# Strong-AI-Lab/ct-vae

Measured on AMD Instinct MI355X. Metric: images/sec/GPU fwd+bwd, 64×64×3 bs=64; recon+KL vs CPU ref, higher is better.
Workload: dtype f32; 1 GPU; VanillaVAE 64x64x3 train step fwd+loss+bwd+Adam (configs/vae.yaml shapes at the batch BASELINE.json's metric names, bs=64, on one MI355X; BASELINE.json configs[1..4] are the `configs` entries); per_gpu_batch=64, global_batch=64, latent_dim=128, parallelism=single, hipgraph=True, allreduce_overlap=False

## Files before the change

ct-vae_amd/csrc/api.hip:

```cpp
#include "../../include/ctvae_hip.h"

#include "common.hpp"
#include "gatlayer.hpp"
#include "glinear.hpp"
#include "pair.hpp"

namespace ctvae {
int launch_tapgemm(const ConvGeom& g, const float* G, const float* W, const float* bias, const float* add,
                   const float* mask, int mask_act, float* S, int act, float* bn_part, float* ws, size_t ws_floats,
                   hipStream_t st, const BnBwdFuse* bnb = nullptr, const InXform* xf = nullptr,
                   const WinoFilters* wf = nullptr, SplitKRaw* raw = nullptr, int out_pix = 0);
bool out_pix_supported(const ConvGeom& g, size_t ws_floats, int out_pix);
bool wino_supported(const ConvGeom& g, size_t ws_floats);
bool wino_enabled();
int wino_set_enabled(int on);
int launch_crop_resize_u8(const unsigned char* img, const long long* rows, float* out, int B, int N, int H, int W, int crop,
                          int S, hipStream_t st);
bool thin_forward_supported(const ConvGeom& g);
bool thin_wgrad_supported(const ConvGeom& g);
int tapgemm_bnb_rows(const ConvGeom& g, size_t ws_floats);
bool img_dgrad_supported(const ConvGeom& g);
void tapgemm_plan(const ConvGeom& g, size_t ws_floats, TapGemmPlan& p);
int launch_wgrad(const ConvGeom& g, const float* X, const float* dY, float* dW, float* dbias, float* ws, size_t ws_bytes,
                 int accumulate, hipStream_t st, const InXform* xf = nullptr, const DyXform* dyx = nullptr);
// ... 338 lines not shown
  const InXform xf{in_scale, in_shift, in_act};
  const InXform* xfp = in_scale != nullptr ? &xf : nullptr;
  if (!a_out && !scale_shift_out) return kErrBadArg;
  if (training && (!save_mean || !save_invstd)) return kErrBadArg;
  if (!training && (!running_mean || !running_var)) return kErrBadArg;
  if (Co % 4 != 0) return kErrBadArg;
  ConvGeom g;
  if (conv_geom(g, kind, 0, B, H, W, Ci, Co, k, stride, pad, out_pad)) return kErrBadArg;
  const size_t wsf = ws_bytes / sizeof(float);
  TapGemmPlan plan;
  tapgemm_plan(g, wsf, plan);
  const int R = g.B * g.sH * g.sW;
  if (plan.splitk > 1 || !training) {
    SplitKRaw raw{ws, 0};
    const bool fused = training && plan.splitk > 1 && bn_fused_ok(R, Co);
    int rc = launch_tapgemm(g, x, w, bias, nullptr, nullptr, 0, y, ACT_NONE, nullptr, ws, wsf, (hipStream_t)stream, nullptr, xfp,
                            nullptr, fused ? &raw : nullptr);
    if (rc) return rc;
    if (raw.splitk > 1) {
      const BnFusedFwd p{ws, row_map_of(g), raw.splitk, R, Co, bias, gamma, beta, running_mean, running_var, momentum, eps, save_mean, save_invstd,
                         scale_shift_out, nbt, y, a_out, act};
      return launch_bn_fused_forward(p, (hipStream_t)stream);
    }
    return launch_bn_forward(y, R, Co, gamma, beta, running_mean, running_var, momentum, eps, training, act, a_out, save_mean,
                             save_invstd, ws, ws_bytes, nbt, (hipStream_t)stream, scale_shift_out);
  }
  const int nparts = plan.bn_parts;
  if (wsf < bn_workspace_floats(Co, nparts)) return kErrWorkspace;
  int rc = launch_tapgemm(g, x, w, bias, nullptr, nullptr, 0, y, ACT_NONE, ws, nullptr, 0, (hipStream_t)stream, nullptr, xfp);
  if (rc) return rc;
  return launch_bn_finish_forward(y, R, Co, nparts, gamma, beta, running_mean, running_var, momentum, eps, training, act,
                                  a_out, save_mean, save_invstd, ws, nbt, (hipStream_t)stream, scale_shift_out);
}

int ctvae_conv_dgrad(int kind, const float* dy, const float* w, const float* add, const float* mask, int mask_act,
                     float* dx, int B, int H, int W, int Ci, int Co, int k, int stride, int pad, int out_pad,
                     const float* wino_filters, float* ws, size_t ws_bytes, void* stream) {
  if (!dy || !w || !dx || !conv_kind_ok(kind)) return kErrBadArg;
  ConvGeom g;
  if (conv_geom(g, kind, 2, B, H, W, Ci, Co, k, stride, pad, out_pad)) return kErrBadArg;
  if (wino_filters != nullptr && !ctvae_conv_wino_filter_floats(kind, B, H, W, Ci, Co, k, stride, pad, out_pad, ws_bytes))
    return kErrBadArg;
  const WinoFilters wf{wino_filters, nullptr};
  return launch_tapgemm(g, dy, w, nullptr, add, mask, mask_act, dx, ACT_NONE, nullptr, ws, ws_bytes / sizeof(float),
                        (hipStream_t)stream, nullptr, nullptr, &wf);
}

int ctvae_conv_wgrad(int kind, const float* x, const float* dy, float* dw, float* dbias, int B, int H, int W, int Ci,
                     int Co, int k, int stride, int pad, int out_pad, int accumulate, const float* in_scale,
                     const float* in_shift, int in_act, const float* dy_bn_y, const float* dy_bn_coef, int dy_bn_act,
                     float* gy_out, float* bn_dgamma, float* bn_dbeta, int bn_accumulate, float* ws, size_t ws_bytes,
                     void* stream) {
  if (!x || !dy || !dw || !ws || !conv_kind_ok(kind)) return kErrBadArg;
  if ((in_scale != nullptr) != (in_shift != nullptr)) return kErrBadArg;
  if ((dy_bn_y != nullptr) != (dy_bn_coef != nullptr) || (gy_out != nullptr && dy_bn_y == nullptr)) return kErrBadArg;
  if ((bn_dgamma != nullptr) != (bn_dbeta != nullptr) || (bn_dgamma != nullptr && (dy_bn_y == nullptr || gy_out != nullptr)))
    return kErrBadArg;
  ConvGeom g;
  if (conv_geom(g, kind, 0, B, H, W, Ci, Co, k, stride, pad, out_pad)) return kErrBadArg;
  const InXform xf{in_scale, in_shift, in_act};
  const DyXform dyx{dy_bn_y, dy_bn_coef, gy_out, dy_bn_act, bn_dgamma, bn_dbeta, bn_accumulate};
  float* wws = defer_wgrad_ws(ws, ws_bytes / sizeof(float));
  const int rc = launch_wgrad(g, x, dy, dw, dbias, wws, ws_bytes, accumulate, (hipStream_t)stream, &xf, &dyx);
  defer_wgrad_done();
  return rc;
}

int ctvae_defer_begin(float* arena, size_t arena_bytes) { return defer_begin(arena, arena_bytes / sizeof(float)); }
int ctvae_defer_flush(void* stream) { return defer_flush((hipStream_t)stream); }

int ctvae_conv_backward_bn_rows(int kind, int B, int H, int W, int Ci, int Co, int k, int stride, int pad, int out_pad,
                                size_t ws_bytes) {
  if (!conv_kind_ok(kind)) return 0;
  ConvGeom g;
  if (conv_geom(g, kind, 2, B, H, W, Ci, Co, k, stride, pad, out_pad)) return 0;
  PairCtx ctx;
  pair_ctx() = &ctx;
  const int rows = tapgemm_bnb_rows(g, ((ws_bytes / 2) & ~(size_t)255) / sizeof(float));
  pair_ctx() = nullptr;
  return rows;
}

static thread_local int g_lazy_pixel_major = 0;

static int conv_backward_impl(int kind, const float* x, const float* dy, const float* w, float* dw, float* dbias, float* dx, int B,
                        int H, int W, int Ci, int Co, int k, int stride, int pad, int out_pad, int accumulate, const float* mask,
                        int mask_act, const float* wino_filters, const float* bn_y, const float* bn_mean,
                        const float* bn_invstd, const float* bn_gamma, const float* bn_beta, int bn_act, float* bn_part,
                        int bn_part_rows, float* bn_coef_out, float* bn_dgamma, float* bn_dbeta, int bn_accumulate,
                        const float* in_scale, const float* in_shift, int in_act,
                        const float* dy_bn_y, const float* dy_bn_coef, int dy_bn_act, float* gy_out, float* ws, size_t ws_bytes,
                        void* stream, float* dx_slices) {
  if (!x || !dy || !w || !dw || (!dx && !dx_slices) || !ws || !conv_kind_ok(kind)) return kErrBadArg;
  const bool bn = bn_part != nullptr;
  if (bn_coef_out != nullptr && !bn) return kErrBadArg;
  if ((bn_dgamma != nullptr) != (bn_dbeta != nullptr) || (bn_dgamma != nullptr && bn_coef_out == nullptr)) return kErrBadArg;
  if ((in_scale != nullptr) != (in_shift != nullptr)) return kErrBadArg;
  if ((dy_bn_y != nullptr) != (dy_bn_coef != nullptr) || (dy_bn_y != nullptr) != (gy_out != nullptr)) return kErrBadArg;
  if (bn && (!bn_y || !bn_mean || !bn_invstd || !bn_gamma || !bn_beta)) return kErrBadArg;
  ConvGeom gw, gd;
  if (conv_geom(gw, kind, 0, B, H, W, Ci, Co, k, stride, pad, out_pad)) return kErrBadArg;
  if (conv_geom(gd, kind, 2, B, H, W, Ci, Co, k, stride, pad, out_pad)) return kErrBadArg;
  const size_t half_bytes = (ws_bytes / 2) & ~(size_t)255, half_floats = half_bytes / sizeof(float);
  float* ws_d = ws + half_floats;
  if (wino_filters != nullptr && !ctvae_conv_wino_filter_floats(kind, B, H, W, Ci, Co, k, stride, pad, out_pad, half_bytes))
    return kErrBadArg;
  const hipStream_t st = (hipStream_t)stream;
  PairCtx ctx;
  pair_ctx() = &ctx;
  if (bn) {
    const int rows = tapgemm_bnb_rows(gd, half_floats);
    if (rows <= 0 || rows != bn_part_rows || (img_dgrad_supported(gd) && mask != nullptr)) {
      pair_ctx() = nullptr;
      return kErrBadArg;
    }
  }
  {
    TapGemmPlan pl;
    tapgemm_plan(gd, half_floats, pl);
    ctx.dgrad_wgs = (long)pl.mtiles * pl.ntiles * gd.ncls * (pl.splitk > 1 ? pl.splitk : 1);
    int kmax = 0;
    for (int c = 0; c < gd.ncls; ++c) kmax = gd.ntaps[c] * gd.gC / KC > kmax ? gd.ntaps[c] * gd.gC / KC : kmax;
    ctx.dgrad_chunks = pl.splitk > 1 ? (kmax + pl.splitk - 1) / pl.splitk : kmax;
  }
  const InXform xf{in_scale, in_shift, in_act};
  const DyXform dyx{dy_bn_y, dy_bn_coef, gy_out, dy_bn_act};
  int rc;
  if (bn && bn_act != ACT_TANH && x == bn_y && in_scale != nullptr && in_act == bn_act && mask == nullptr && dy_bn_y == nullptr &&
      img_conv_supported(gw) && img_dgrad_supported(gd) && img_backward_fused_ws_floats(gd) <= half_floats) {
    float *part = nullptr, *pb = nullptr;
    int np = 0;
    const BnBwdFuse f{bn_y, bn_mean, bn_invstd, bn_gamma, bn_beta, bn_act, bn_part};
    rc = launch_img_backward_fused(gd, dy, w, dx, &f, ws, &part, &pb, &np, dbias != nullptr, st);
    if (!rc) rc = wgrad_finish_slabs(part, dw, 9L * 32 * 3, np, pb, dbias, 3L, accumulate, st);
  } else {
    float* wws = bn_coef_out == nullptr ? defer_wgrad_ws(ws, half_floats) : ws;
    rc = launch_wgrad(gw, x, dy, dw, dbias, wws, half_bytes, accumulate, st, &xf, &dyx);
    defer_wgrad_done();
    if (!rc) {
    const WinoFilters wf{wino_filters, nullptr};
    const BnBwdFuse f{bn_y, bn_mean, bn_invstd, bn_gamma, bn_beta, bn_act, bn_part};
      SplitKRaw raw{dx_slices, 0, g_lazy_pixel_major};
      g_lazy_pixel_major = 0;
      rc = launch_tapgemm(gd, gy_out != nullptr ? gy_out : dy, w, nullptr, nullptr, mask, mask_act, dx, ACT_NONE, nullptr, ws_d,
                          half_floats, st, bn ? &f : nullptr, nullptr, &wf, dx_slices != nullptr ? &raw : nullptr);
      if (!rc && dx_slices != nullptr && raw.splitk <= 1) rc = kErrBadArg;
    }
  }
  pair_ctx() = nullptr;
  if (rc) return rc;
  if (bn_coef_out != nullptr) {
    ctx.haveBF = true;
    ctx.bf = BnFinJob{bn_part, bn_part_rows, Ci, (float)((long)B * H * W), bn_gamma, bn_mean, bn_invstd, bn_beta, bn_coef_out,
                      bn_dgamma, bn_dbeta, bn_accumulate};
  }
  return pair_flush(ctx, st);
}

int ctvae_conv_backward(int kind, const float* x, const float* dy, const float* w, float* dw, float* dbias, float* dx, int B,
                        int H, int W, int Ci, int Co, int k, int stride, int pad, int out_pad, int accumulate, const float* mask,
                        int mask_act, const float* wino_filters, const float* bn_y, const float* bn_mean,
                        const float* bn_invstd, const float* bn_gamma, const float* bn_beta, int bn_act, float* bn_part,
                        int bn_part_rows, float* bn_coef_out, float* bn_dgamma, float* bn_dbeta, int bn_accumulate,
                        const float* in_scale, const float* in_shift, int in_act,
                        const float* dy_bn_y, const float* dy_bn_coef, int dy_bn_act, float* gy_out, float* ws, size_t ws_bytes,
                        void* stream) {
  return conv_backward_impl(kind, x, dy, w, dw, dbias, dx, B, H, W, Ci, Co, k, stride, pad, out_pad, accumulate, mask, mask_act,
                            wino_filters, bn_y, bn_mean, bn_invstd, bn_gamma, bn_beta, bn_act, bn_part, bn_part_rows, bn_coef_out,
                            bn_dgamma, bn_dbeta, bn_accumulate, in_scale, in_shift, in_act, dy_bn_y, dy_bn_coef, dy_bn_act, gy_out, ws,
                            ws_bytes, stream, nullptr);
}

int ctvae_conv_backward_lazy_slices(int kind, int B, int H, int W, int Ci, int Co, int k, int stride, int pad, int out_pad,
                                    int for_bn, size_t ws_bytes) {
  if (!conv_kind_ok(kind)) return 0;
  ConvGeom g;
  if (conv_geom(g, kind, 2, B, H, W, Ci, Co, k, stride, pad, out_pad)) return 0;
  const size_t half_floats = ((ws_bytes / 2) & ~(size_t)255) / sizeof(float);
  if (img_dgrad_supported(g) || (wino_enabled() && wino_supported(g, half_floats))) return 0;
  PairCtx ctx;
  pair_ctx() = &ctx;
  TapGemmPlan pl;
  tapgemm_plan(g, half_floats, pl);
  pair_ctx() = nullptr;
  const long Mc = (long)g.B * g.Qh * g.Qw;
  if (pl.thin || pl.splitk <= 1) return 0;
  if (for_bn && (Mc % 4 != 0 || !bn_fused_ok(B * H * W, Ci))) return 0;
  return pl.splitk;
}

int ctvae_conv_backward_lazy(int kind, const float* x, const float* dy, const float* w, float* dw, float* dbias, float* dx_slices,
                             int B, int H, int W, int Ci, int Co, int k, int stride, int pad, int out_pad, int accumulate,
                             const float* in_scale, const float* in_shift, int in_act, int pixel_major, float* ws, size_t ws_bytes,
                             void* stream) {
  if (!dx_slices) return kErrBadArg;
  g_lazy_pixel_major = pixel_major;
  return conv_backward_impl(kind, x, dy, w, dw, dbias, nullptr, B, H, W, Ci, Co, k, stride, pad, out_pad, accumulate, nullptr, 0,
                            nullptr, nullptr, nullptr, nullptr, nullptr, nullptr, 0, nullptr, 0, nullptr, nullptr, nullptr, 0, in_scale,
                            in_shift, in_act, nullptr, nullptr, 0, nullptr, ws, ws_bytes, stream, dx_slices);
}

int ctvae_bn_backward_fused(const float* g_a_slices, int slices, int kind, int B, int H, int W, int Ci, int Co, int k, int stride,
                            int pad, int out_pad, const float* y, const float* gamma, const float* beta, const float* save_mean,
                            const float* save_invstd, int act, float* g_y, float* dgamma, float* dbeta, int accumulate, void* stream) {
  if (!g_a_slices || slices < 1 || !y || !gamma || !beta || !save_mean || !save_invstd || !g_y || !dgamma || !dbeta) return kErrBadArg;
  if (!conv_kind_ok(kind)) return kErrBadArg;
  ConvGeom g;
  if (conv_geom(g, kind, 2, B, H, W, Ci, Co, k, stride, pad, out_pad)) return kErrBadArg;
  const BnFusedBwd p{g_a_slices, row_map_of(g), slices, B * H * W, Ci, y, gamma, beta, save_mean, save_invstd, act, g_y, dgamma,
                     dbeta, accumulate};
  return launch_bn_fused_backward(p, (hipStream_t)stream);
}

int ctvae_conv_wgrad_bn_apply_supported(int kind, int B, int H, int W, int Ci, int Co, int k, int stride, int pad, int out_pad) {
  if (!conv_kind_ok(kind)) return 0;
  ConvGeom g;
  if (conv_geom(g, kind, 0, B, H, W, Ci, Co, k, stride, pad, out_pad)) return 0;
  if (upconv_wgrad_supported(g)) return 1;
  return img_enc_supported(g) ? 2 : 0;
}

int ctvae_bn_forward(const float* y, int R, int C, const float* gamma, const float* beta, float* running_mean,
                     float* running_var, float momentum, float eps, int training, int act, float* out,
                     float* save_mean, float* save_invstd, int64_t* num_batches_tracked, float* ws, size_t ws_bytes,
                     void* stream) {
  if (!y || !gamma || !beta || !out || !ws) return kErrBadArg;
  if (training && (!save_mean || !save_invstd)) return kErrBadArg;
  if (!training && (!running_mean || !running_var)) return kErrBadArg;
  return launch_bn_forward(y, R, C, gamma, beta, running_mean, running_var, momentum, eps, training, act, out, save_mean,
                           save_invstd, ws, ws_bytes, (long long*)num_batches_tracked, (hipStream_t)stream);
}

int ctvae_bn_backward(const float* g_a, const float* beta, const float* y, int R, int C, const float* gamma,
                      const float* save_mean, const float* save_invstd, int act, float* g_y, float* dgamma,
                      float* dbeta, int accumulate, const float* part_in, int part_rows, float* coef_out,
                      const float* coef_in, float* ws, size_t ws_bytes, void* stream) {
  if (!g_a || !beta || !y || !gamma || !save_mean || !save_invstd || !dgamma || !dbeta || !ws) return kErrBadArg;
  if (!g_y && !coef_out) return kErrBadArg;
  if ((part_in != nullptr) != (part_rows > 0)) return kErrBadArg;
  if (coef_in != nullptr && (!g_y || part_in != nullptr || coef_out != nullptr)) return kErrBadArg;
  return launch_bn_backward(g_a, beta, y, R, C, gamma, save_mean, save_invstd, act, g_y, dgamma, dbeta, accumulate, ws,
                            ws_bytes, part_in, part_rows, (hipStream_t)stream, coef_out, coef_in);
}

int ctvae_gat_score(int mode, const float* xl, const float* xr, const float* attr, const float* we, const float* att, float* out,
                    int B, int N, int H, int C, float slope, void* stream) {
  if (!xl || !xr || !attr || !we || !att || !out || (mode != 0 && mode != 1)) return kErrBadArg;
  return launch_gat_score(mode, xl, xr, attr, we, att, out, B, N, H, C, slope, (hipStream_t)stream);
}

int ctvae_gat_score_backward(const float* xl, const float* xr, const float* attr, const float* we, const float* att,
                             const float* g, float* d_xl, float* d_xr, float* d_att_part, float* d_we_part, int B, int N, int H,
                             int C, float slope, void* stream) {
  if (!xl || !xr || !attr || !we || !att || !g || !d_xl || !d_xr || !d_att_part || !d_we_part) return kErrBadArg;
  return launch_gat_score_backward(xl, xr, attr, we, att, g, d_xl, d_xr, d_att_part, d_we_part, B, N, H, C, slope,
// ... 678 lines not shown
```

ct-vae_amd/csrc/common.hpp:

```cpp
#pragma once
#include <hip/hip_runtime.h>
#include <stdint.h>
#include <stdio.h>
#include <string.h>

#include "geom.hpp"

namespace ctvae {

typedef float f32x2 __attribute__((ext_vector_type(2)));
typedef float f32x4 __attribute__((ext_vector_type(4)));
typedef float f32x16 __attribute__((ext_vector_type(16)));

constexpr float kLeaky = 0.01f;

enum Act : int { ACT_NONE = 0, ACT_LRELU = 1, ACT_RELU = 2, ACT_TANH = 3 };

__device__ __forceinline__ float act_fwd(float v, int act) {
  switch (act) {
    case ACT_LRELU: return v > 0.f ? v : v * kLeaky;
    case ACT_RELU: return v > 0.f ? v : 0.f;
    case ACT_TANH: return 1.f - 2.f * __frcp_rn(__expf(2.f * v) + 1.f);
    default: return v;
  }
// ... 31 lines not shown
}

__device__ __forceinline__ double wave_sum_d_full(double v) {
#define CTVAE_DPP_D(CTRL, RM, BC)                                                                          \
  {                                                                                                        \
    const long long b = __builtin_bit_cast(long long, v);                                                  \
    const int lo = __builtin_amdgcn_update_dpp(0, (int)b, CTRL, RM, 0xF, BC);                               \
    const int hi = __builtin_amdgcn_update_dpp(0, (int)(b >> 32), CTRL, RM, 0xF, BC);                       \
    v += __builtin_bit_cast(double, ((long long)hi << 32) | (unsigned)lo);                                 \
  }
  CTVAE_DPP_D(0xB1, 0xF, true)
  CTVAE_DPP_D(0x4E, 0xF, true)
  CTVAE_DPP_D(0x141, 0xF, true)
  CTVAE_DPP_D(0x140, 0xF, true)
  CTVAE_DPP_D(0x142, 0xA, false)
  CTVAE_DPP_D(0x143, 0xC, false)
#undef CTVAE_DPP_D
  const long long b = __builtin_bit_cast(long long, v);
  const int lo = __builtin_amdgcn_readlane((int)b, 63), hi = __builtin_amdgcn_readlane((int)(b >> 32), 63);
  return __builtin_bit_cast(double, ((long long)hi << 32) | (unsigned)lo);
}

__device__ __forceinline__ double wave_sum_d(double v) {
#pragma unroll
  for (int o = 32; o > 0; o >>= 1) v += __shfl_xor(v, o, 64);
  return v;
}

__device__ __forceinline__ float block_sum_256(float v, float* sm ) {
  v = wave_sum_full(v);
  const int w = threadIdx.x >> 6;
  __syncthreads();
  if ((threadIdx.x & 63) == 0) sm[w] = v;
  __syncthreads();
  return sm[0] + sm[1] + sm[2] + sm[3];
}

inline int ceil_div(int a, int b) { return (a + b - 1) / b; }

template <int BYTES>
__device__ __forceinline__ void kernarg_warm() {
#if defined(__HIP_DEVICE_COMPILE__)
  const void* ka = __builtin_amdgcn_kernarg_segment_ptr();
  unsigned junk;
  asm volatile(
      ".set .Lkw_off, 0\n"
      ".rept %2\n"
      "s_load_dword %0, %1, .Lkw_off\n"
      ".set .Lkw_off, .Lkw_off + 64\n"
      ".endr\n"
      "s_waitcnt lgkmcnt(0)"
      : "=&s"(junk)
      : "s"(ka), "n"((BYTES + 63) / 64)
      : "memory");
#endif
}
template <int BYTES, int O0, int O1, int O2>
__device__ __forceinline__ void kernarg_warm_get(int& v0, int& v1, int& v2) {
#if defined(__HIP_DEVICE_COMPILE__)
  const void* ka = __builtin_amdgcn_kernarg_segment_ptr();
  unsigned junk;
  asm volatile(
      "s_load_dword %1, %4, %6\n"
      "s_load_dword %2, %4, %7\n"
      "s_load_dword %3, %4, %8\n"
      ".set .Lkw_off, 0\n"
      ".rept %5\n"
      "s_load_dword %0, %4, .Lkw_off\n"
      ".set .Lkw_off, .Lkw_off + 64\n"
      ".endr\n"
      "s_waitcnt lgkmcnt(0)"
      : "=&s"(junk), "=&s"(v0), "=&s"(v1), "=&s"(v2)
      : "s"(ka), "n"((BYTES + 63) / 64), "n"(O0), "n"(O1), "n"(O2)
      : "memory");
#endif
}

struct InXform {
  const float* scale;
  const float* shift;
  int act;
};

struct DyXform {
  const float* y;
  const float* coef;
  float* gy_out;
  int act;
  float* dgamma = nullptr;
  float* dbeta = nullptr;
  int bn_accumulate = 0;
};

struct WinoFilters {
  const float* ready;
  float* bwd_out;
};

struct BnBwdFuse {
  const float* y;
  const float* mean;
  const float* invstd;
  const float* gamma;
  const float* beta;
  int act;
  float* part;
};

struct SplitKRaw {
  float* part;
  int splitk;
  int pixel_major = 0;
};

struct RowMap {
  int ncls, Mc, Qh, Qw, sH, sW, os;
  unsigned pyp, pxp;
  int lgMc, lgQhw, lgQw;
};

inline RowMap row_map_of(const ConvGeom& g) {
  RowMap m{};
  m.ncls = g.ncls; m.Mc = g.B * g.Qh * g.Qw; m.Qh = g.Qh; m.Qw = g.Qw; m.sH = g.sH; m.sW = g.sW; m.os = g.os;
  static_assert(kMaxCls <= 4, "RowMap packs four classes");
  for (int c = 0; c < kMaxCls; ++c) { m.pyp |= (unsigned)(g.py[c] & 0xff) << (8 * c); m.pxp |= (unsigned)(g.px[c] & 0xff) << (8 * c); }
  auto lg2 = [](int v) { int l = 0; while ((1 << l) < v) ++l; return (v > 0 && (1 << l) == v) ? l : -1; };
  m.lgMc = lg2(m.Mc); m.lgQhw = lg2(g.Qh * g.Qw); m.lgQw = lg2(g.Qw);
  if (m.lgMc < 0 || m.lgQhw < 0 || m.lgQw < 0) m.lgMc = m.lgQhw = m.lgQw = -1;
  return m;
}

__device__ __forceinline__ int row_map_pixel(const RowMap& m, int r) {
  if (m.ncls == 1) return r;
  int cls, b, qy, qx;
  if (m.lgMc >= 0) {
    cls = r >> m.lgMc;
    const int mm = r & (m.Mc - 1);
    b = mm >> m.lgQhw;
    const int rr = mm & ((1 << m.lgQhw) - 1);
    qy = rr >> m.lgQw;
    qx = rr & (m.Qw - 1);
  } else {
    cls = r / m.Mc;
    const int mm = r - cls * m.Mc;
    const int qhw = m.Qh * m.Qw;
    b = mm / qhw;
    const int rr = mm - b * qhw;
    qy = rr / m.Qw;
    qx = rr - qy * m.Qw;
  }
  const int py = (int)((m.pyp >> (8 * cls)) & 0xffu), px = (int)((m.pxp >> (8 * cls)) & 0xffu);
  return (b * m.sH + qy * m.os + py) * m.sW + qx * m.os + px;
}

struct TapGemmPlan {
  int BM, BN, mtiles, ntiles, splitk;
  int thin;
  int bn_parts;
};

#define CTVAE_LAUNCH_CHECK()                   \
  do {                                         \
    hipError_t e__ = hipGetLastError();        \
    if (e__ != hipSuccess) return (int)e__;    \
  } while (0)

constexpr int kErrBadArg = -22;
constexpr int kErrWorkspace = -12;

}
```

ct-vae_amd/csrc/image.hip:

```cpp
#include <type_traits>

#include "common.hpp"
#include "prof.hpp"

namespace ctvae {

#ifdef CTVAE_PHASE_TIMING
__device__ unsigned long long g_img_phase[1024 * 32];
#define IPHASE(i) do { if (threadIdx.x == 0 && blockIdx.x < 1024 && (i) < 32) g_img_phase[blockIdx.x * 32 + (i)] = wall_clock64(); } while (0)
extern "C" int ctvae_debug_img_phase_read(unsigned long long* out, int n) {
  return (int)hipMemcpyFromSymbol(out, HIP_SYMBOL(g_img_phase), (size_t)n * 8);
}
#else
#define IPHASE(i) do {} while (0)
#endif

namespace {

constexpr int TH = 8, TW = 32, PH = 10, PW = 34, NP = PH * PW , NPP = 352 ;
constexpr int LDA = 36;
constexpr int GH = 12, GW = 36;
constexpr int C = 32, NO = 3, NT = 9, NJ = 27;
constexpr unsigned kOOBi = 0x80000000u;

// ... 397 lines not shown
  auto g_load = [&](const TileXY& t) {
#pragma unroll
    for (int j = 0; j < 2; ++j) {
      const int pp = tid + 256 * j;
      const int py = (pp * 241) >> 13, px = pp - py * PW;
      const int iy = t.y0 - 1 + py, ix = t.x0 - 1 + px;
      const bool ok = pp < NP && (unsigned)iy < (unsigned)a.H && (unsigned)ix < (unsigned)a.W;
      const unsigned off = ok ? (unsigned)(((t.b * a.H + iy) * a.W + ix) * NO) * 4u : kOOBi;
#pragma unroll
      for (int n = 0; n < NO; ++n) gq[j][n] = ld1(rG, ok ? off + 4u * n : kOOBi);
    }
  };
  int tile = blockIdx.x;
  TileXY cur = tile_xy(a, tile < a.ntiles ? tile : 0);
  if (tile < a.ntiles) g_load(cur);
  for (; tile < a.ntiles; tile += gridDim.x) {
#pragma unroll
    for (int j = 0; j < 2; ++j) {
      const int pp = tid + 256 * j;
      if (pp < NP)
#pragma unroll
        for (int n = 0; n < NO; ++n) sG[pp * 4 + n] = gq[j][n];
    }
    __syncthreads();
    const int next = tile + gridDim.x;
    const TileXY nxt = tile_xy(a, next < a.ntiles ? next : 0);
    if (next < a.ntiles) g_load(nxt);
#pragma unroll
    for (int i = 0; i < 2; ++i) {
      const int ly = wave + 4 * i;
      const unsigned rowoff = (unsigned)(((cur.b * a.H + cur.y0 + ly) * a.W + cur.x0) * C + li) * 4u;
      float yv[16];
      if (bn) {
#pragma unroll
        for (int r = 0; r < 16; ++r) yv[r] = ld1(rY, rowoff + (unsigned)((8 * (r >> 2) + 4 * lh + (r & 3)) * C) * 4u);
      }
      f32x16 acc;
#pragma unroll
      for (int r = 0; r < 16; ++r) acc[r] = 0.f;
      const float* gp = &sG[((ly + 1) * PW + li + 1) * 4];
#pragma unroll
      for (int s = 0; s < 14; ++s) acc = __builtin_amdgcn_mfma_f32_32x32x2f32(gp[koff[s]], bw[s], acc, 0, 0, 0);
#pragma unroll
      for (int r = 0; r < 16; ++r) st1(rO, rowoff + (unsigned)((8 * (r >> 2) + 4 * lh + (r & 3)) * C) * 4u, acc[r]);
      if (bn) {
        if (a.bn_act == ACT_TANH) {
#pragma unroll
          for (int r = 0; r < 16; ++r) {
            const float xh = (yv[r] - bmean) * binv;
            const float g1 = acc[r] * act_bwd_from_out(act_fwd(bgm * xh + bbt, ACT_TANH), ACT_TANH);
            s1 += g1;
            s2 += g1 * xh;
          }
        } else {
          const float bsl = act_slope(a.bn_act);
#pragma unroll
          for (int r = 0; r < 16; ++r) {
            const float xh = (yv[r] - bmean) * binv;
            const float g1 = acc[r] * act_slope_bwd(bgm * xh + bbt, bsl);
            s1 += g1;
            s2 += g1 * xh;
          }
        }
      }
    }
    __syncthreads();
    cur = nxt;
  }
  if (bn) {
    s1 += __shfl_xor(s1, 32, 64);
    s2 += __shfl_xor(s2, 32, 64);
    if (lh == 0) {
      sS[(wave * C + li) * 2] = s1;
      sS[(wave * C + li) * 2 + 1] = s2;
    }
    __syncthreads();
    if (tid < C * 2) {
      const float v = ((sS[tid] + sS[C * 2 + tid]) + sS[2 * C * 2 + tid]) + sS[3 * C * 2 + tid];
      a.bn_part[(long)blockIdx.x * C * 2 + tid] = v;
    }
  }
}

__global__ __launch_bounds__(256, 4) void img_bwd_fused_kernel(const ImgArgs a, float* __restrict__ wpart, float* __restrict__ wpbias) {
  kernarg_warm<sizeof(ImgArgs) + 16>();
  const float bn_slope = act_slope(a.bn_act);
  __shared__ __attribute__((aligned(16))) float sG[NP * 4];
  __shared__ __attribute__((aligned(16))) float sR[4 * 32 * 32];
  __shared__ float sS[4 * C * 2];
  __shared__ float sB[4 * NO];
  const int tid = threadIdx.x, lane = tid & 63, wave = tid >> 6, li = lane & 31, lh = lane >> 5;
  const __amdgpu_buffer_rsrc_t rG = rsrc(a.dY, (long)a.B * a.H * a.W * NO * 4);
  const long obytes = (long)a.B * a.H * a.W * C * 4;
  const __amdgpu_buffer_rsrc_t rO = rsrc(a.out, obytes);
  const __amdgpu_buffer_rsrc_t rY = rsrc(a.bn_y, obytes);

  int koff[14];
  float bw[14];
#pragma unroll
  for (int s = 0; s < 14; ++s) {
    const int k0 = 2 * s, k1 = 2 * s + 1;
    const int t0 = k0 / 3, c0 = k0 % 3, t1 = (k1 < NJ ? k1 : 0) / 3, c1 = (k1 < NJ ? k1 : 0) % 3;
    const int o0 = (a.tdy[t0] * PW + a.tdx[t0]) * 4 + c0, o1 = (a.tdy[t1] * PW + a.tdx[t1]) * 4 + c1;
    const float w0 = a.Wt[(a.twt[t0] * C + li) * NO + c0];
    const float w1 = k1 < NJ ? a.Wt[(a.twt[t1] * C + li) * NO + c1] : 0.f;
    koff[s] = lh ? (k1 < NJ ? o1 : 0) : o0;
    bw[s] = lh ? w1 : w0;
  }
  const int jj = li < NJ ? li : NJ - 1;
  const int t_l = jj / 3, co_l = jj - 3 * t_l;
  const int wlane = ((1 + tap_dy(a, t_l)) * PW + (1 + tap_dx(a, t_l)) + 4 * lh) * 4 + co_l;
  const float bmean = a.bn_mean[li], binv = a.bn_invstd[li], bgm = a.bn_gamma[li], bbt = a.bn_beta[li];
  float s1 = 0.f, s2 = 0.f;
  float bs[NO] = {0.f, 0.f, 0.f};
  f32x16 wacc;
#pragma unroll
  for (int r = 0; r < 16; ++r) wacc[r] = 0.f;

  float gq[2][NO];
  auto g_load = [&](const TileXY& t) {
#pragma unroll
    for (int j = 0; j < 2; ++j) {
      const int pp = tid + 256 * j;
      const int py = (pp * 241) >> 13, px = pp - py * PW;
      const int iy = t.y0 - 1 + py, ix = t.x0 - 1 + px;
      const bool ok = pp < NP && (unsigned)iy < (unsigned)a.H && (unsigned)ix < (unsigned)a.W;
      const unsigned off = ok ? (unsigned)(((t.b * a.H + iy) * a.W + ix) * NO) * 4u : kOOBi;
#pragma unroll
      for (int n = 0; n < NO; ++n) gq[j][n] = ld1(rG, ok ? off + 4u * n : kOOBi);
    }
  };
  int tile = blockIdx.x;
  TileXY cur = tile_xy(a, tile < a.ntiles ? tile : 0);
  if (tile < a.ntiles) g_load(cur);
  for (; tile < a.ntiles; tile += gridDim.x) {
#pragma unroll
    for (int j = 0; j < 2; ++j) {
      const int pp = tid + 256 * j;
      if (pp < NP) {
        const int py = (pp * 241) >> 13, px = pp - py * PW;
        const bool inner = py >= 1 && py <= TH && px >= 1 && px <= TW;
#pragma unroll
        for (int n = 0; n < NO; ++n) {
          sG[pp * 4 + n] = gq[j][n];
          bs[n] += inner ? gq[j][n] : 0.f;
        }
      }
    }
    __syncthreads();
    const int next = tile + gridDim.x;
    const TileXY nxt = tile_xy(a, next < a.ntiles ? next : 0);
    if (next < a.ntiles) g_load(nxt);
#pragma unroll 1
    for (int i = 0; i < 2; ++i) {
      const int ly = wave + 4 * i;
      const unsigned rowoff = (unsigned)(((cur.b * a.H + cur.y0 + ly) * a.W + cur.x0) * C + li) * 4u;
      float yv[16];
#pragma unroll
      for (int r = 0; r < 16; ++r) yv[r] = ld1(rY, rowoff + (unsigned)((8 * (r >> 2) + 4 * lh + (r & 3)) * C) * 4u);
      f32x16 acc;
#pragma unroll
      for (int r = 0; r < 16; ++r) acc[r] = 0.f;
      const float* gp = &sG[((ly + 1) * PW + li + 1) * 4];
#pragma unroll
      for (int s = 0; s < 14; ++s) acc = __builtin_amdgcn_mfma_f32_32x32x2f32(gp[koff[s]], bw[s], acc, 0, 0, 0);
#pragma unroll
      for (int r = 0; r < 16; ++r) st1(rO, rowoff + (unsigned)((8 * (r >> 2) + 4 * lh + (r & 3)) * C) * 4u, acc[r]);
      const float* gw = &sG[ly * PW * 4 + wlane];
#pragma unroll
      for (int r = 0; r < 16; ++r) {
        const float xh = (yv[r] - bmean) * binv;
        const float t = bgm * xh + bbt;
        const float av = act_slope_fwd(t, bn_slope);
        const float g1 = acc[r] * act_slope_bwd(t, bn_slope);
        s1 += g1;
        s2 += g1 * xh;
        wacc = __builtin_amdgcn_mfma_f32_32x32x2f32(av, gw[(8 * (r >> 2) + (r & 3)) * 4], wacc, 0, 0, 0);
      }
    }
    __syncthreads();
    cur = nxt;
  }
  s1 += __shfl_xor(s1, 32, 64);
  s2 += __shfl_xor(s2, 32, 64);
  if (lh == 0) {
    sS[(wave * C + li) * 2] = s1;
    sS[(wave * C + li) * 2 + 1] = s2;
  }
#pragma unroll
  for (int r = 0; r < 16; ++r) sR[(wave * 32 + 8 * (r >> 2) + 4 * lh + (r & 3)) * 32 + li] = wacc[r];
  float bwv[NO];
#pragma unroll
  for (int n = 0; n < NO; ++n) bwv[n] = wave_sum(bs[n]);
  if (lane == 0)
#pragma unroll
    for (int n = 0; n < NO; ++n) sB[wave * NO + n] = bwv[n];
  __syncthreads();
  if (tid < C * 2) {
    const float v = ((sS[tid] + sS[C * 2 + tid]) + sS[2 * C * 2 + tid]) + sS[3 * C * 2 + tid];
    a.bn_part[(long)blockIdx.x * C * 2 + tid] = v;
  }
  for (int e = tid; e < C * NJ; e += 256) {
    const int ci = e / NJ, j = e - ci * NJ;
    const float v = ((sR[(0 * 32 + ci) * 32 + j] + sR[(1 * 32 + ci) * 32 + j]) + sR[(2 * 32 + ci) * 32 + j]) + sR[(3 * 32 + ci) * 32 + j];
    const int t = j / 3, co = j - 3 * t;
    wpart[((long)blockIdx.x * (NT * C) + tap_wt(a, t) * C + ci) * NO + co] = v;
  }
  if (wpbias != nullptr && tid < NO) wpbias[(long)blockIdx.x * NO + tid] = ((sB[tid] + sB[NO + tid]) + sB[2 * NO + tid]) + sB[3 * NO + tid];
}

constexpr int EPH = 2 * TH + 1, EPW = 2 * TW + 1, ENP = EPH * EPW;
constexpr int ENLD = (ENP + 255) / 256;

struct EncArgs {
  const float* X;
  const float* Wt;
  const float* bias;
  const float* dY;
  float* out;
  float* pbias;
  float* bn_part;
  const float* dy_y;
  const float* dy_coef;
  float* dgamma;
  float* dbeta;
  int dy_act, bn_accumulate;
  int act;
  int B, H, W, tiles_y, tiles_x, ntiles;
  int tdy[NT], tdx[NT], twt[NT];
};

struct EncPatch {
  float v[ENLD][NO];
};

__device__ __forceinline__ void enc_patch_load(const EncArgs& a, __amdgpu_buffer_rsrc_t rX, const TileXY& t, EncPatch& p) {
  const int IH = 2 * a.H, IW = 2 * a.W;
#pragma unroll
  for (int j = 0; j < ENLD; ++j) {
    const int pp = threadIdx.x + 256 * j;
    const int py = (pp * 1009) >> 16, px = pp - py * EPW;
    const int iy = 2 * t.y0 - 1 + py, ix = 2 * t.x0 - 1 + px;
    const bool ok = pp < ENP && (unsigned)iy < (unsigned)IH && (unsigned)ix < (unsigned)IW;
    const unsigned off = (unsigned)(((t.b * IH + iy) * IW + ix) * NO) * 4u;
#pragma unroll
    for (int n = 0; n < NO; ++n) p.v[j][n] = ld1(rX, ok ? off + 4u * n : kOOBi);
  }
}
__device__ __forceinline__ void enc_patch_store(const EncPatch& p, float* sX) {
#pragma unroll
// ... 246 lines not shown
  ProfScope ps("img_enc_fwd_kernel", st, 2.0 * a.ntiles * TH * TW * NT * C * NO, 4.0 * a.ntiles * TH * TW * (C + 4 * NO));
  hipLaunchKernelGGL(img_enc_fwd_kernel, dim3(img_enc_rows(g)), dim3(256), 0, st, a);
  CTVAE_LAUNCH_CHECK();
  return 0;
}

int launch_img_enc_wgrad(const ConvGeom& g, const float* X, const float* dY, float* ws, float** part_out, float** pbias_out,
                         int* nparts, bool want_bias, hipStream_t st, const DyXform* dyx) {
  EncArgs a{};
  fill_enc(a, g);
  a.X = X; a.dY = dY;
  if (dyx != nullptr && dyx->y != nullptr) {
    if (dyx->gy_out != nullptr || (dyx->act != ACT_NONE && dyx->act != ACT_RELU && dyx->act != ACT_LRELU)) return kErrBadArg;
    if ((dyx->dgamma != nullptr) != (dyx->dbeta != nullptr)) return kErrBadArg;
    a.dy_y = dyx->y; a.dy_coef = dyx->coef; a.dy_act = dyx->act;
    a.dgamma = dyx->dgamma; a.dbeta = dyx->dbeta; a.bn_accumulate = dyx->bn_accumulate;
  }
  const int nwg = a.ntiles < 512 ? a.ntiles : 512;
  a.out = ws;
  a.pbias = want_bias ? ws + (size_t)nwg * NJ * C : nullptr;
  ProfScope ps("img_enc_wgrad_kernel", st, 2.0 * a.ntiles * TH * TW * NT * C * NO, 4.0 * a.ntiles * TH * TW * (C + 4 * NO));
  if (a.dy_y != nullptr) hipLaunchKernelGGL(img_enc_wgrad_kernel<true>, dim3(nwg), dim3(256), 0, st, a);
  else hipLaunchKernelGGL(img_enc_wgrad_kernel<false>, dim3(nwg), dim3(256), 0, st, a);
  CTVAE_LAUNCH_CHECK();
  *part_out = a.out;
  *pbias_out = a.pbias;
  *nparts = nwg;
  return 0;
}

constexpr int kImgFwd2Wgs = 1024, kImgWgradWgs = 512, kImgDgradWgs = 1024;

int img_wgrad_parts(const ConvGeom& g) {
  const int nt = g.B * (g.sH / TH) * (g.sW / TW);
  return nt < kImgWgradWgs ? nt : kImgWgradWgs;
}
int img_dgrad_rows(const ConvGeom& g) {
  const int nt = g.B * (g.sH / TH) * (g.sW / TW);
  return nt < kImgDgradWgs ? nt : kImgDgradWgs;
}

int launch_img_forward(const ConvGeom& g, const float* X, const float* W, const float* bias, float* S, int act,
                       const InXform* xf, hipStream_t st) {
  ImgArgs a{};
  fill(a, g);
  a.X = X; a.Wt = W; a.bias = bias; a.out = S; a.act = act;
  if (xf != nullptr && xf->scale != nullptr) { a.scale = xf->scale; a.shift = xf->shift; a.in_act = xf->act; }
  ProfScope ps("img_fwd_kernel", st, 2.0 * a.ntiles * TH * TW * NT * C * NO, 4.0 * a.ntiles * TH * TW * (C + NO));
  const int nwg = a.ntiles < kImgFwd2Wgs ? a.ntiles : kImgFwd2Wgs;
  hipLaunchKernelGGL(img_fwd2_kernel, dim3(nwg), dim3(256), 0, st, a);
  CTVAE_LAUNCH_CHECK();
  return 0;
}

int launch_img_wgrad(const ConvGeom& g, const float* X, const float* dY, float* ws, float** part_out, float** pbias_out,
                     int* nparts, bool want_bias, const InXform* xf, hipStream_t st) {
  ImgArgs a{};
  fill(a, g);
  a.X = X; a.dY = dY;
  if (xf != nullptr && xf->scale != nullptr) { a.scale = xf->scale; a.shift = xf->shift; a.in_act = xf->act; }
  const int nwg = img_wgrad_parts(g);
  a.out = ws;
  a.pbias = want_bias ? ws + (size_t)nwg * NT * C * NO : nullptr;
  ProfScope ps("img_wgrad_kernel", st, 2.0 * a.ntiles * TH * TW * NT * C * NO, 4.0 * a.ntiles * TH * TW * (C + NO));
  hipLaunchKernelGGL(img_wgrad_kernel, dim3(nwg), dim3(256), 0, st, a);
  CTVAE_LAUNCH_CHECK();
  *part_out = a.out;
  *pbias_out = a.pbias;
  *nparts = nwg;
  return 0;
}

int launch_img_backward_fused(const ConvGeom& g, const float* dY, const float* W, float* dX, const BnBwdFuse* bnb, float* ws,
                              float** part_out, float** pbias_out, int* nparts, bool want_bias, hipStream_t st) {
  if (bnb->act == ACT_TANH) return kErrBadArg;
  ImgArgs a{};
  fill(a, g);
  a.dY = dY; a.Wt = W; a.out = dX;
  a.bn_y = bnb->y; a.bn_mean = bnb->mean; a.bn_invstd = bnb->invstd; a.bn_gamma = bnb->gamma; a.bn_beta = bnb->beta;
  a.bn_act = bnb->act; a.bn_part = bnb->part;
  const int nwg = img_dgrad_rows(g);
  float* part = ws;
  float* pb = want_bias ? ws + (size_t)nwg * NT * C * NO : nullptr;
  ProfScope ps("img_bwd_fused_kernel", st, 4.0 * a.ntiles * TH * TW * NT * C * NO, 4.0 * a.ntiles * TH * TW * (C * 2 + NO));
  hipLaunchKernelGGL(img_bwd_fused_kernel, dim3(nwg), dim3(256), 0, st, a, part, pb);
  CTVAE_LAUNCH_CHECK();
  *part_out = part;
  *pbias_out = pb;
  *nparts = nwg;
  return 0;
}
size_t img_backward_fused_ws_floats(const ConvGeom& g) { return (size_t)img_dgrad_rows(g) * (NT * C * NO + NO); }

int launch_img_dgrad(const ConvGeom& g, const float* dY, const float* W, float* dX, const BnBwdFuse* bnb, hipStream_t st) {
  ImgArgs a{};
  fill(a, g);
  a.dY = dY; a.Wt = W; a.out = dX;
  if (bnb != nullptr && bnb->part != nullptr) {
    a.bn_y = bnb->y; a.bn_mean = bnb->mean; a.bn_invstd = bnb->invstd; a.bn_gamma = bnb->gamma; a.bn_beta = bnb->beta;
    a.bn_act = bnb->act; a.bn_part = bnb->part;
  }
  const int nwg = img_dgrad_rows(g);
  ProfScope ps("img_dgrad_kernel", st, 2.0 * a.ntiles * TH * TW * NT * C * NO,
               4.0 * a.ntiles * TH * TW * (C * (a.bn_part != nullptr ? 2 : 1) + NO));
  hipLaunchKernelGGL(img_dgrad_kernel, dim3(nwg), dim3(256), 0, st, a);
  CTVAE_LAUNCH_CHECK();
  return 0;
}

}
```

ct-vae_amd/csrc/upconv.hip:

```cpp
#include "common.hpp"
#include "phase.hpp"
#include <type_traits>

#include "prof.hpp"

namespace ctvae {

namespace {

constexpr int TH = 8, TW = 32, PH = 9, PW = 33, NP = PH * PW ;
constexpr int LDA = 36, C = 32, NT = 9, NCLS = 4, MAXT = 4;
constexpr int NLD = (NP * 8 + 255) / 256;
constexpr unsigned kOOBu = 0x80000000u;

struct UpArgs {
  const float* X;
  const float* Wt;
  const float* bias;
  const float* dY;
  float* out;
  float* pbias;
  float* bn_part;
  const float* dy_y;
  const float* dy_coef;
  float* gy_out;
  int dy_act;
  const float* xf_scale;
  const float* xf_shift;
  int xf_act;
  int act;
  int B, H, W, tiles_y, tiles_x, ntiles;
  int ntaps[NCLS], cpy[NCLS], cpx[NCLS];
  int tdy[NCLS][MAXT], tdx[NCLS][MAXT], twt[NCLS][MAXT];
};

__device__ __forceinline__ f32x4 ld4(__amdgpu_buffer_rsrc_t r, unsigned off) {
  return __builtin_bit_cast(f32x4, __builtin_amdgcn_raw_buffer_load_b128(r, (int)off, 0, 0));
}
__device__ __forceinline__ float ld1(__amdgpu_buffer_rsrc_t r, unsigned off) {
  return __builtin_bit_cast(float, __builtin_amdgcn_raw_buffer_load_b32(r, (int)off, 0, 0));
}
__device__ __forceinline__ void st1(__amdgpu_buffer_rsrc_t r, unsigned off, float v) {
  __builtin_amdgcn_raw_buffer_store_b32(__builtin_bit_cast(unsigned, v), r, (int)off, 0, 0);
}
__device__ __forceinline__ __amdgpu_buffer_rsrc_t rsrc(const void* p, long bytes) {
  return __builtin_amdgcn_make_buffer_rsrc(const_cast<void*>(p), 0, (int)bytes, 0x00020000);
}

struct TileXY {
  int b, y0, x0;
};
__device__ __forceinline__ TileXY tile_xy(const UpArgs& a, int tile) {
  const int per = a.tiles_y * a.tiles_x;
  const int b = tile / per, r = tile - b * per;
  const int ty = r / a.tiles_x;
  return TileXY{b, ty * TH, (r - ty * a.tiles_x) * TW};
}

struct Patch {
  f32x4 v[NLD];
};
__device__ __forceinline__ void patch_load(const UpArgs& a, __amdgpu_buffer_rsrc_t rX, const TileXY& t, Patch& p) {
#pragma unroll
  for (int j = 0; j < NLD; ++j) {
    const int e = threadIdx.x + 256 * j;
    const int pp = e >> 3, c4 = e & 7;
    const int py = (pp * 1986) >> 16, px = pp - py * PW;
    const int iy = t.y0 + py, ix = t.x0 + px;
    const bool ok = e < NP * 8 && iy < a.H && ix < a.W;
    p.v[j] = ld4(rX, ok ? (unsigned)(((t.b * a.H + iy) * a.W + ix) * C + 4 * c4) * 4u : kOOBu);
  }
}
__device__ __forceinline__ void patch_store(const Patch& p, float* sA) {
#pragma unroll
  for (int j = 0; j < NLD; ++j) {
    const int e = threadIdx.x + 256 * j;
    if (e < NP * 8) *reinterpret_cast<f32x4*>(&sA[(e >> 3) * LDA + 4 * (e & 7)]) = p.v[j];
  }
}
__device__ __forceinline__ void patch_store_xf(const UpArgs& a, const TileXY& t, const Patch& p, float* sA, f32x4 sc, f32x4 sh,
                                               float nslope) {
#pragma unroll
  for (int j = 0; j < NLD; ++j) {
    const int e = threadIdx.x + 256 * j;
    const int pp = e >> 3;
    const int py = (pp * 1986) >> 16, px = pp - py * PW;
    const float inside = (t.y0 + py < a.H && t.x0 + px < a.W) ? 1.f : 0.f;
    f32x4 v = p.v[j];
#pragma unroll
    for (int q = 0; q < 4; ++q) {
      const float u = v[q] * sc[q] + sh[q] * inside;
      v[q] = fmaxf(u, u * nslope);
    }
    if (e < NP * 8) *reinterpret_cast<f32x4*>(&sA[pp * LDA + 4 * (e & 7)]) = v;
  }
}

CTVAE_PHASE_DECL(up)
__global__ __launch_bounds__(256, 2) void up_fwd_kernel(const UpArgs a) {
  CTVAE_PH(up, 0, 0);
  kernarg_warm<sizeof(UpArgs)>();
  extern __shared__ __attribute__((aligned(16))) float smem[];
  float* sA = smem;
  float* sW = smem + NP * LDA;
  __shared__ float sS[4 * C * 3];
  const int tid = threadIdx.x, lane = tid & 63, wave = tid >> 6, li = lane & 31, lh = lane >> 5;
  const __amdgpu_buffer_rsrc_t rX = rsrc(a.X, (long)a.B * a.H * a.W * C * 4);
  const int OH = 2 * a.H, OW = 2 * a.W;
  const __amdgpu_buffer_rsrc_t rO = rsrc(a.out, (long)a.B * OH * OW * C * 4);
// ... 78 lines not shown
    auto zero = [](f32x16& acc) {
#pragma unroll
      for (int r = 0; r < 16; ++r) acc[r] = 0.f;
    };
#define UP_STEP(LY, C_, T_, CUR, NXT, NLY, NC, NT_, HAS_NEXT)          \
    if (HAS_NEXT) read_tap(NLY, NC, NT_, NXT);                          \
    mfma_tap(CUR, acc);                                                 \
    _Pragma("unroll") for (int g_ = 0; g_ < 16; ++g_) {                 \
      __builtin_amdgcn_sched_group_barrier(0x008, 1, 0);                \
      __builtin_amdgcn_sched_group_barrier(0x100, 2, 0);                \
    }                                                                   \
    __builtin_amdgcn_sched_barrier(0);
    Frag fa, fb;
#pragma unroll 1
    for (int i = 0; i < 2; ++i) {
      const int ly = wave + 4 * i;
      f32x16 acc;
      read_tap(ly, 0, 0, fa);
      zero(acc);
      UP_STEP(ly, 0, 0, fa, fb, ly, 1, 0, true)
      epilogue(ly, 0, acc);
      zero(acc);
      UP_STEP(ly, 1, 0, fb, fa, ly, 1, 1, true)
      UP_STEP(ly, 1, 1, fa, fb, ly, 2, 0, true)
      epilogue(ly, 1, acc);
      zero(acc);
      UP_STEP(ly, 2, 0, fb, fa, ly, 2, 1, true)
      UP_STEP(ly, 2, 1, fa, fb, ly, 3, 0, true)
      epilogue(ly, 2, acc);
      zero(acc);
      UP_STEP(ly, 3, 0, fb, fa, ly, 3, 1, true)
      UP_STEP(ly, 3, 1, fa, fb, ly, 3, 2, true)
      UP_STEP(ly, 3, 2, fb, fa, ly, 3, 3, true)
      UP_STEP(ly, 3, 3, fa, fb, ly, 0, 0, false)
      epilogue(ly, 3, acc);
    }
#undef UP_STEP
    CTVAE_PH(up, 0, 3);
    __syncthreads();
    CTVAE_PH(up, 0, 4);
    cur = nxt;
  }
  if (a.bn_part != nullptr) {
    {
      const float on = __shfl_xor(sn, 32, 64), om = __shfl_xor(smean, 32, 64), oq = __shfl_xor(sm2, 32, 64);
      const float ntot = sn + on;
      if (ntot > 0.f) {
        const float d = om - smean;
        sm2 = sm2 + oq + d * d * (sn * on / ntot);
        smean = smean + d * (on / ntot);
      }
      sn = ntot;
    }
    if (lh == 0) {
      float* st = &sS[(wave * C + li) * 3];
      st[0] = sn; st[1] = smean; st[2] = sm2;
    }
    __syncthreads();
    if (tid < C) {
      float n = 0.f, mean = 0.f, m2 = 0.f;
#pragma unroll
      for (int w = 0; w < 4; ++w) {
        const float nb = sS[(w * C + tid) * 3], mb = sS[(w * C + tid) * 3 + 1], qb = sS[(w * C + tid) * 3 + 2];
        if (nb > 0.f) {
          const float ntot = n + nb, d = mb - mean;
          mean += d * (nb / ntot);
          m2 += qb + d * d * (n * nb / ntot);
          n = ntot;
        }
      }
      float* p = a.bn_part + ((long)blockIdx.x * C + tid) * 3;
      p[0] = n; p[1] = mean; p[2] = m2;
    }
  }
}


template <int CLS>
struct ClsInfo {
  static constexpr int ntaps = CLS == 0 ? 1 : (CLS == 3 ? 4 : 2);
  static constexpr int first = CLS == 0 ? 0 : (CLS == 1 ? 1 : (CLS == 2 ? 3 : 5));
};

template <bool FUSED>
__global__ __launch_bounds__(256, 1) void up_wgrad_kernel(const UpArgs a) {
  kernarg_warm<sizeof(UpArgs)>();
  __shared__ __attribute__((aligned(16))) float sA[NP * LDA];
  __shared__ __attribute__((aligned(16))) float sR[4 * C * C];
  __shared__ float sB[4 * C];
  const int tid = threadIdx.x, lane = tid & 63, wave = tid >> 6, li = lane & 31, lh = lane >> 5;
  const __amdgpu_buffer_rsrc_t rX = rsrc(a.X, (long)a.B * a.H * a.W * C * 4);
  const int OH = 2 * a.H, OW = 2 * a.W;
  const long obytes = (long)a.B * OH * OW * C * 4;
  const __amdgpu_buffer_rsrc_t rG = rsrc(a.dY, obytes);
  const __amdgpu_buffer_rsrc_t rYb = rsrc(a.dy_y, FUSED ? obytes : 0);
  const __amdgpu_buffer_rsrc_t rGY = rsrc(a.gy_out, FUSED ? obytes : 0);
  const float k1 = FUSED ? a.dy_coef[li] : 0.f, k2 = FUSED ? a.dy_coef[C + li] : 0.f, k3 = FUSED ? a.dy_coef[2 * C + li] : 0.f;
  const float ksc = FUSED ? a.dy_coef[3 * C + li] : 0.f, ksh = FUSED ? a.dy_coef[4 * C + li] : 0.f;
  const float nslope = a.dy_act == ACT_LRELU ? kLeaky : (a.dy_act == ACT_RELU ? 0.f : 1.f);
  const bool xf = a.xf_scale != nullptr;
  const f32x4 xsc = xf ? *reinterpret_cast<const f32x4*>(a.xf_scale + 4 * (tid & 7)) : f32x4{0.f, 0.f, 0.f, 0.f};
  const f32x4 xsh = xf ? *reinterpret_cast<const f32x4*>(a.xf_shift + 4 * (tid & 7)) : f32x4{0.f, 0.f, 0.f, 0.f};
  const float xns = a.xf_act == ACT_LRELU ? kLeaky : (a.xf_act == ACT_RELU ? 0.f : 1.f);

  f32x16 acc[NT];
#pragma unroll
  for (int t = 0; t < NT; ++t)
#pragma unroll
    for (int r = 0; r < 16; ++r) acc[t][r] = 0.f;
  float bsum = 0.f;

  CTVAE_PH(up, 1, 0);
  for (int tile = blockIdx.x; tile < a.ntiles; tile += gridDim.x) {
    const TileXY cur = tile_xy(a, tile);
    CTVAE_PH(up, 1, 1);
#pragma unroll
    for (int h = 0; h < 2; ++h) {
      f32x4 v[NLD / 2];
#pragma unroll
      for (int j = 0; j < NLD / 2; ++j) {
        const int e = tid + 256 * (j + h * (NLD / 2));
        const int pp = e >> 3, c4 = e & 7;
        const int py = (pp * 1986) >> 16, px = pp - py * PW;
        const int iy = cur.y0 + py, ix = cur.x0 + px;
        const bool ok = e < NP * 8 && iy < a.H && ix < a.W;
        v[j] = ld4(rX, ok ? (unsigned)(((cur.b * a.H + iy) * a.W + ix) * C + 4 * c4) * 4u : kOOBu);
      }
      if (xf) {
#pragma unroll
        for (int j = 0; j < NLD / 2; ++j) {
          const int e = tid + 256 * (j + h * (NLD / 2));
          const int pp = e >> 3;
          const int py = (pp * 1986) >> 16, px = pp - py * PW;
          const float inside = (cur.y0 + py < a.H && cur.x0 + px < a.W) ? 1.f : 0.f;
#pragma unroll
          for (int q = 0; q < 4; ++q) {
            const float u = v[j][q] * xsc[q] + xsh[q] * inside;
            v[j][q] = fmaxf(u, u * xns);
          }
        }
      }
#pragma unroll
      for (int j = 0; j < NLD / 2; ++j) {
        const int e = tid + 256 * (j + h * (NLD / 2));
        if (e < NP * 8) *reinterpret_cast<f32x4*>(&sA[(e >> 3) * LDA + 4 * (e & 7)]) = v[j];
      }
    }
    __syncthreads();

    CTVAE_PH(up, 1, 2);
    float dv[3][8], yv[FUSED ? 3 : 1][FUSED ? 8 : 1];
    auto step_off = [&](int ly, int c, int h) {
      return (unsigned)((((cur.b * OH + 2 * (cur.y0 + ly) + a.cpy[c]) * OW + 2 * cur.x0 + a.cpx[c] + 2 * (16 * h + lh)) * C + li)) * 4u;
    };
    auto dy_load = [&](unsigned off, auto slot_c) {
      constexpr int slot = decltype(slot_c)::value;
#pragma unroll
      for (int j = 0; j < 8; ++j) dv[slot][j] = ld1(rG, off + (unsigned)(4 * j * C) * 4u);
      if constexpr (FUSED) {
#pragma unroll
        for (int j = 0; j < 8; ++j) yv[slot][j] = ld1(rYb, off + (unsigned)(4 * j * C) * 4u);
      }
    };
    auto run_step = [&](int ly, auto cls_c, int h, unsigned off, auto slot_c) {
      constexpr int CLS = decltype(cls_c)::value;
      constexpr int slot = decltype(slot_c)::value;
      using CI = ClsInfo<CLS>;
      int xo[CI::ntaps];
#pragma unroll
      for (int t = 0; t < CI::ntaps; ++t) xo[t] = ((ly + a.tdy[CLS][t]) * PW + 16 * h + lh + a.tdx[CLS][t]) * LDA + li;
      float xa[CI::ntaps], xb[CI::ntaps];
#pragma unroll
      for (int t = 0; t < CI::ntaps; ++t) xa[t] = sA[xo[t]];
#pragma unroll
      for (int j = 0; j < 8; ++j) {
        if (j + 1 < 8) {
#pragma unroll
          for (int t = 0; t < CI::ntaps; ++t) xb[t] = sA[xo[t] + 2 * (j + 1) * LDA];
        }
        float d = dv[slot][j];
        if constexpr (FUSED) {
          const float yy = yv[slot][j];
          const float g1 = (yy * ksc + ksh) > 0.f ? d : d * nslope;
          d = k1 * g1 + k2 * yy + k3;
          st1(rGY, off + (unsigned)(4 * j * C) * 4u, d);
        }
        bsum += d;
#pragma unroll
        for (int t = 0; t < CI::ntaps; ++t)
          acc[CI::first + t] = __builtin_amdgcn_mfma_f32_32x32x2f32(xa[t], d, acc[CI::first + t], 0, 0, 0);
#pragma unroll
        for (int t = 0; t < CI::ntaps; ++t) xa[t] = xb[t];
        __builtin_amdgcn_sched_barrier(0);
      }
    };
    unsigned soff[3];
    auto issue = [&](auto s_c) {
      constexpr int S = decltype(s_c)::value;
      soff[S % 3] = step_off(wave + 4 * (S / 8), (S % 8) / 2, S & 1);
      dy_load(soff[S % 3], std::integral_constant<int, S % 3>{});
    };
    auto do_step = [&](auto s_c) {
      constexpr int S = decltype(s_c)::value;
      if constexpr (S + 2 < 16) issue(std::integral_constant<int, S + 2>{});
      run_step(wave + 4 * (S / 8), std::integral_constant<int, (S % 8) / 2>{}, S & 1, soff[S % 3], std::integral_constant<int, S % 3>{});
    };
    issue(std::integral_constant<int, 0>{});
    issue(std::integral_constant<int, 1>{});
#define UPW_STEP(S_) do_step(std::integral_constant<int, S_>{});
    UPW_STEP(0) UPW_STEP(1) UPW_STEP(2) UPW_STEP(3) UPW_STEP(4) UPW_STEP(5) UPW_STEP(6) UPW_STEP(7)
    CTVAE_PH(up, 1, 3);
    UPW_STEP(8) UPW_STEP(9) UPW_STEP(10) UPW_STEP(11) UPW_STEP(12) UPW_STEP(13) UPW_STEP(14) UPW_STEP(15)
#undef UPW_STEP
    CTVAE_PH(up, 1, 4);
    __syncthreads();
  }
  bsum += __shfl_xor(bsum, 32, 64);
  if (lh == 0) sB[wave * C + li] = bsum;
  auto merge_tap = [&](int wtap, const f32x16& v) {
    __syncthreads();
#pragma unroll
    for (int r = 0; r < 16; ++r) sR[(wave * C + 8 * (r >> 2) + 4 * lh + (r & 3)) * C + li] = v[r];
    __syncthreads();
    for (int e = tid; e < C * C; e += 256) {
      const float s4 = ((sR[e] + sR[C * C + e]) + sR[2 * C * C + e]) + sR[3 * C * C + e];
      a.out[((long)blockIdx.x * NT + wtap) * C * C + e] = s4;
    }
  };
  merge_tap(a.twt[0][0], acc[0]);
  merge_tap(a.twt[1][0], acc[1]);
  merge_tap(a.twt[1][1], acc[2]);
  merge_tap(a.twt[2][0], acc[3]);
  merge_tap(a.twt[2][1], acc[4]);
  merge_tap(a.twt[3][0], acc[5]);
  merge_tap(a.twt[3][1], acc[6]);
  merge_tap(a.twt[3][2], acc[7]);
  merge_tap(a.twt[3][3], acc[8]);
  if (a.pbias != nullptr && tid < C) a.pbias[(long)blockIdx.x * C + tid] = ((sB[tid] + sB[C + tid]) + sB[2 * C + tid]) + sB[3 * C + tid];
  CTVAE_PH(up, 1, 5);
}

void fill(UpArgs& a, const ConvGeom& g) {
  a.B = g.B; a.H = g.gH; a.W = g.gW;
  a.tiles_y = g.gH / TH; a.tiles_x = g.gW / TW;
  a.ntiles = g.B * a.tiles_y * a.tiles_x;
  for (int c = 0; c < NCLS; ++c) {
    a.ntaps[c] = g.ntaps[c]; a.cpy[c] = g.py[c]; a.cpx[c] = g.px[c];
    for (int t = 0; t < MAXT; ++t) {
      const bool ok = t < g.ntaps[c];
      a.tdy[c][t] = ok ? g.taps[c][t].dy : 0;
      a.tdx[c][t] = ok ? g.taps[c][t].dx : 0;
      a.twt[c][t] = ok ? g.taps[c][t].wtap : 0;
    }
  }
}

constexpr size_t kUpFwdSmem = (size_t)(NP * LDA + NT * C * C) * 4;

}

bool upconv_supported(const ConvGeom& g) {
  if (!packed_weights(g) || g.wT != 0 || g.gC != C || g.sC != C || g.wCi != C || g.wCo != C) return false;
  if (g.is != 1 || g.os != 2 || g.ncls != NCLS) return false;
  if (g.sH != 2 * g.gH || g.sW != 2 * g.gW || g.gH % TH != 0 || g.gW % TW != 0) return false;
  int total = 0;
  for (int c = 0; c < NCLS; ++c) {
    if (g.ntaps[c] < 1 || g.ntaps[c] > MAXT) return false;
    total += g.ntaps[c];
    for (int t = 0; t < g.ntaps[c]; ++t) {
      const Tap& tp = g.taps[c][t];
      if (tp.dy < 0 || tp.dy > 1 || tp.dx < 0 || tp.dx > 1 || tp.wtap < 0 || tp.wtap >= NT) return false;
    }
  }
  if (g.ntaps[0] != 1 || g.ntaps[1] != 2 || g.ntaps[2] != 2 || g.ntaps[3] != 4) return false;
  return total == NT && (long)g.B * g.sH * g.sW * C < (1L << 29);
}
bool upconv_wgrad_supported(const ConvGeom& g) { return upconv_supported(g); }

constexpr int kUpWgs = 512;
int upconv_rows(const ConvGeom& g) {
  const int nt = g.B * (g.gH / TH) * (g.gW / TW);
  return nt < kUpWgs ? nt : kUpWgs;
}

int launch_upconv_forward(const ConvGeom& g, const float* X, const float* W, const float* bias, float* S, int act,
                          float* bn_part, hipStream_t st, const InXform* xf) {
  UpArgs a{};
  fill(a, g);
  a.X = X; a.Wt = W; a.bias = bias; a.out = S; a.act = act; a.bn_part = bn_part;
  if (xf != nullptr && xf->scale != nullptr) {
    if (xf->act != ACT_NONE && xf->act != ACT_RELU && xf->act != ACT_LRELU) return kErrBadArg;
    a.xf_scale = xf->scale; a.xf_shift = xf->shift; a.xf_act = xf->act;
  }
  static bool attr_set = false;
  if (!attr_set) {
    (void)hipFuncSetAttribute(reinterpret_cast<const void*>(up_fwd_kernel), hipFuncAttributeMaxDynamicSharedMemorySize, (int)kUpFwdSmem);
    attr_set = true;
  }
  ProfScope ps("up_fwd_kernel", st, 2.0 * a.ntiles * TH * TW * NT * C * C, 4.0 * a.ntiles * TH * TW * C * 5.0);
  hipLaunchKernelGGL(up_fwd_kernel, dim3(upconv_rows(g)), dim3(256), kUpFwdSmem, st, a);
  CTVAE_LAUNCH_CHECK();
  return 0;
}

int launch_upconv_wgrad(const ConvGeom& g, const float* X, const float* dY, float* ws, float** part_out, float** pbias_out,
                        int* nparts, bool want_bias, hipStream_t st, const DyXform* dyx, const InXform* xf) {
  UpArgs a{};
  fill(a, g);
  a.X = X; a.dY = dY;
  if (xf != nullptr && xf->scale != nullptr) {
    if (xf->act != ACT_NONE && xf->act != ACT_RELU && xf->act != ACT_LRELU) return kErrBadArg;
    a.xf_scale = xf->scale; a.xf_shift = xf->shift; a.xf_act = xf->act;
  }
  if (dyx != nullptr && dyx->y != nullptr && dyx->act != ACT_NONE && dyx->act != ACT_RELU && dyx->act != ACT_LRELU) return kErrBadArg;
  if (dyx != nullptr && dyx->y != nullptr) { a.dy_y = dyx->y; a.dy_coef = dyx->coef; a.gy_out = dyx->gy_out; a.dy_act = dyx->act; }
  const int nwg = upconv_rows(g);
  a.out = ws;
  a.pbias = want_bias ? ws + (size_t)nwg * NT * C * C : nullptr;
  ProfScope ps("up_wgrad_kernel", st, 2.0 * a.ntiles * TH * TW * NT * C * C, 4.0 * a.ntiles * TH * TW * C * 5.0);
  if (a.dy_y != nullptr) hipLaunchKernelGGL(up_wgrad_kernel<true>, dim3(nwg), dim3(256), 0, st, a);
  else hipLaunchKernelGGL(up_wgrad_kernel<false>, dim3(nwg), dim3(256), 0, st, a);
  CTVAE_LAUNCH_CHECK();
  *part_out = a.out;
  *pbias_out = a.pbias;
  *nparts = nwg;
  return 0;
}

}
```

ct-vae_amd/csrc/wgrad.hip:

```cpp
#include "common.hpp"
#include "prof.hpp"
#include "finish.hpp"
#include "pair.hpp"
#include "wgrad_fast.hpp"

namespace ctvae {


template <int WK, int WN, bool XVEC, bool DVEC>
__global__ __launch_bounds__(256) void wgrad_kernel(const WgradArgs a) {
  kernarg_warm<sizeof(WgradArgs)>();
  __shared__ __attribute__((aligned(16))) float sXbuf[MC * WK * 32];
  __shared__ __attribute__((aligned(16))) float sDbuf[MC * WN * 32];
  __shared__ int sRowPix[2][MC];
  __shared__ int sRowYX[2][MC];
  __shared__ int sRowOut[2][MC];
  wgrad_plain_body<WK, WN, XVEC, DVEC>(a, sXbuf, sDbuf, sRowPix, sRowYX, sRowOut, blockIdx.x, blockIdx.y, gridDim.x, gridDim.y);
}

template <int WK, int WN, int TK, int TN, bool XF = false>
__global__ __launch_bounds__(256) void wgrad_fast_kernel(const WgradArgs a, int lgQw, int lgQhw, int lgC) {
  kernarg_warm<sizeof(WgradArgs) + 12>();
  constexpr int KT = WK * TK * 32, NT = WN * TN * 32;
  __shared__ __attribute__((aligned(16))) float sX[MC * KT];
// ... 243 lines not shown

static int finish_reduce(const float* p1, float* d1, long n1, int S1, long st1, const float* p2, float* d2, long n2, int S2, long st2,
                         int accumulate, hipStream_t st) {
  if (defer_record(p1, d1, n1, S1, st1, p2, d2, n2, S2, st2, accumulate, st)) return 0;
  if (PairCtx* pc = pair_ctx(); pc != nullptr && !pc->haveRed) {
    pc->j1 = ReduceJob{p1, d1, n1, S1, st1, 0, 0};
    pc->j2 = (p2 != nullptr && d2 != nullptr) ? ReduceJob{p2, d2, n2, S2, st2, 0, 0} : ReduceJob{nullptr, nullptr, 0, 0, 0, 0, 0};
    pc->nb1 = reduce_job_blocks(pc->j1);
    pc->nb2 = reduce_job_blocks(pc->j2);
    pc->accumulate = accumulate;
    pc->bytesRed = 4.0 * (double)(S1 + 1) * n1;
    pc->haveRed = pc->nb1 + pc->nb2 > 0;
    return 0;
  }
  ProfScope ps("reduce_partials_kernel", st, 0.0, 4.0 * (double)(S1 + 1) * n1);
  if (p2 != nullptr && d2 != nullptr) launch_reduce2(p1, d1, n1, S1, st1, p2, d2, n2, S2, st2, accumulate, st);
  else launch_reduce(p1, d1, n1, S1, st1, accumulate, st);
  CTVAE_LAUNCH_CHECK();
  return 0;
}

int wgrad_finish_slabs(const float* part, float* dW, long n, int nparts, const float* pbias, float* dbias, long nb, int accumulate,
                       hipStream_t st) {
  return finish_reduce(part, dW, n, nparts, n, pbias, dbias, nb, nparts, nb, accumulate, st);
}

size_t wgrad_workspace_floats(const ConvGeom& g, int S) {
  int taps_total = 0;
  for (int c = 0; c < g.ncls; ++c) taps_total += g.ntaps[c];
  size_t rows = (size_t)taps_total * g.gC;
  return (size_t)S * rows * g.sC + (size_t)S * g.ncls * g.sC;
}

static int choose_splits(const ConvGeom& g, int KT, int NT, size_t ws_floats, int target_wgs = 1024) {
  int ktiles = 0;
  for (int c = 0; c < g.ncls; ++c) ktiles += ceil_div(g.ntaps[c] * g.gC, KT);
  int tiles = ktiles * ceil_div(g.sC, NT);
  int Mc = g.B * g.Qh * g.Qw;
  int nchunks = ceil_div(Mc, MC);
  int S = target_wgs / (tiles > 0 ? tiles : 1);
  if (S < 1) S = 1;
  const int min_chunks = nchunks >= 32 ? 8 : 4;
  int maxS = ceil_div(nchunks, min_chunks);
  if (maxS < 1) maxS = 1;
  if (S > maxS) S = maxS;
  while (S > 1 && wgrad_workspace_floats(g, S) > ws_floats) --S;
  return S;
}

bool thin_wgrad_supported(const ConvGeom& g);
size_t thin_wgrad_workspace_floats(const ConvGeom& g);
int launch_thin_wgrad(const ConvGeom& g, const float* X, const float* dY, float* ws, float** part_out, float** pbias_out,
                      int* nparts_w, int* nparts_b, bool want_bias, hipStream_t st, const InXform* xf);

bool upconv_wgrad_supported(const ConvGeom& g);
int launch_upconv_wgrad(const ConvGeom& g, const float* X, const float* dY, float* ws, float** part_out, float** pbias_out,
                        int* nparts, bool want_bias, hipStream_t st, const DyXform* dyx, const InXform* xf);
bool img_enc_supported(const ConvGeom& g);
int launch_img_enc_wgrad(const ConvGeom& g, const float* X, const float* dY, float* ws, float** part_out, float** pbias_out,
                         int* nparts, bool want_bias, hipStream_t st, const DyXform* dyx);

bool wino_wgrad_supported(const ConvGeom& g, size_t ws_floats, int* splits);
int launch_wino_wgrad(const ConvGeom& g, const float* X, const float* dY, float* ws, size_t ws_floats, int* nparts,
                      bool want_bias, float** pbias_out, hipStream_t st);

bool wino_enabled();

int launch_wgrad(const ConvGeom& g, const float* X, const float* dY, float* dW, float* dbias, float* ws,
                 size_t ws_bytes, int accumulate, hipStream_t st, const InXform* xf, const DyXform* dyx) {
  if ((xf == nullptr || xf->scale == nullptr) && (dyx == nullptr || dyx->y == nullptr) && wino_enabled() &&
      wino_wgrad_supported(g, ws_bytes / sizeof(float), nullptr)) {
    int np = 0;
    float* pb = nullptr;
    int rc = launch_wino_wgrad(g, X, dY, ws, ws_bytes / sizeof(float), &np, dbias != nullptr, &pb, st);
    if (rc) return rc;
    const long n = 9L * g.gC * g.sC;
    return finish_reduce(ws, dW, n, np, n, pb, dbias, (long)g.sC, np, (long)g.sC, accumulate, st);
  }
  const bool up = upconv_wgrad_supported(g) && ws_bytes / sizeof(float) >= (size_t)512 * (9 * 32 * 32 + 32);
  const bool enc = img_enc_supported(g) && (xf == nullptr || xf->scale == nullptr) &&
                   ws_bytes / sizeof(float) >= (size_t)512 * (27 * 32 + 32);
  if (dyx != nullptr && dyx->y != nullptr && !up && !(enc && dyx->gy_out == nullptr)) return kErrBadArg;
  if (dyx != nullptr && dyx->y != nullptr && up && dyx->gy_out == nullptr) return kErrBadArg;
  if (up) {
    float *part = nullptr, *pb = nullptr;
    int np = 0;
    int rc = launch_upconv_wgrad(g, X, dY, ws, &part, &pb, &np, dbias != nullptr, st, dyx, xf);
    if (rc) return rc;
    const long n = 9L * 32 * 32;
    return finish_reduce(part, dW, n, np, n, pb, dbias, 32L, np, 32L, accumulate, st);
  }
  if (enc) {
    float *part = nullptr, *pb = nullptr;
    int np = 0;
    int rc = launch_img_enc_wgrad(g, X, dY, ws, &part, &pb, &np, dbias != nullptr, st, dyx);
    if (rc) return rc;
    const long n = 27L * 32;
    return finish_reduce(part, dW, n, np, n, pb, dbias, 32L, np, 32L, accumulate, st);
  }
  const bool thin = thin_wgrad_supported(g) && thin_wgrad_workspace_floats(g) <= ws_bytes / sizeof(float);
  const bool has_xf = xf != nullptr && xf->scale != nullptr;
  if (has_xf && !thin && !((g.gC % 4) == 0 && (g.sC % 4) == 0 && g.wT == 0)) return kErrBadArg;
  if (thin) {
    float *part = nullptr, *pb = nullptr;
    int nw = 0, nb = 0;
    int rc = launch_thin_wgrad(g, X, dY, ws, &part, &pb, &nw, &nb, dbias != nullptr, st, xf);
    if (rc) return rc;
    int taps = 0;
    for (int c = 0; c < g.ncls; ++c) taps += g.ntaps[c];
    const long n = (long)taps * g.gC * g.sC;
    return finish_reduce(part, dW, n, nw, n, pb, dbias, (long)g.sC, nb, (long)g.sC, accumulate, st);
  }
  WgradArgs a{};
  a.g = g;
  a.X = X; a.dY = dY;
  a.Mc = g.B * g.Qh * g.Qw;
  a.N = g.sC;
  if (g.wT != 0 || a.Mc <= 0) return kErrBadArg;
  int taps_total = 0;
  for (int c = 0; c < g.ncls; ++c) taps_total += g.ntaps[c];
  a.rows_total = taps_total * g.gC;
  const bool xvec = (g.gC % 4) == 0, dvec = (a.N % 4) == 0;
  const bool narrow = a.N <= 32;
  bool big = !has_xf && xvec && dvec && (a.N % 128) == 0 && a.Mc >= 8192;
  if (has_xf) { a.xf_scale = xf->scale; a.xf_shift = xf->shift; a.xf_act = xf->act; }
  for (int c = 0; c < g.ncls && big; ++c) big = (g.ntaps[c] * g.gC) % 128 == 0;
  if (big) {
    int tiles128 = 0;
    for (int c = 0; c < g.ncls; ++c) tiles128 += g.ntaps[c] * g.gC / 128;
    tiles128 *= a.N / 128;
    big = tiles128 >= 16 && (long)ceil_div(a.Mc, MC) * tiles128 >= 8L * 1024;
  }
  const int KT = big ? 128 : (narrow ? 128 : 64), NT = big ? 128 : (narrow ? 32 : 64);
  const size_t ws_floats = ws_bytes / sizeof(float);
  const PairCtx* pcw = pair_ctx();
  const bool will_pair = pcw != nullptr && !pcw->haveB && xvec && dvec && !big &&
                         (!narrow || (pcw->dgrad_wgs > 0 && pcw->dgrad_wgs < 1024));
  const bool coarse = will_pair && pcw->dgrad_wgs > 0 && pcw->dgrad_wgs < 1024 && pcw->dgrad_chunks >= 12;
  const int S = choose_splits(g, KT, NT, ws_floats, big ? 512 : (coarse ? 768 : 1024));
  if (wgrad_workspace_floats(g, S) > ws_floats) return kErrWorkspace;
  a.S = S;
  const int nchunks = ceil_div(a.Mc, MC);
  a.chunks_per_split = ceil_div(nchunks, S);
  a.part = ws;
  a.pbias = dbias ? ws + (size_t)S * a.rows_total * a.N : nullptr;
  int kt = 0;
  for (int c = 0; c < g.ncls; ++c) {
    a.ktile_start[c] = kt;
    kt += ceil_div(g.ntaps[c] * g.gC, KT);
  }
  a.ktile_start[g.ncls] = kt;
  a.ntiles = ceil_div(a.N, NT);
  dim3 grid(kt * a.ntiles, S), block(256);
  bool recorded = false;
  if (PairCtx* pc = pair_ctx(); will_pair) {
    auto lg2 = [](int v) { int l = 0; while ((1 << l) < v) ++l; return (1 << l) == v ? l : -1; };
    const int lw = lg2(g.Qw), lh2 = lg2(g.Qh);
    pc->haveB = true;
    pc->wkB = narrow ? 4 : 2;
    pc->B = a;
    pc->lgQw = (lw >= 0 && lh2 >= 0) ? lw : -1;
    pc->lgQhw = (lw >= 0 && lh2 >= 0) ? lw + lh2 : -1;
    pc->lgC = lg2(g.gC);
    pc->gxB = grid.x; pc->gyB = grid.y;
    pc->flopsB = 2.0 * (double)a.Mc * a.N * a.rows_total;
    pc->bytesB = 4.0 * ((double)g.B * g.gH * g.gW * g.gC + (double)g.B * g.sH * g.sW * g.sC);
// ... 70 lines not shown
```

ct-vae_amd/kernels.py:

```python
import math
import weakref
from dataclasses import dataclass

import torch
from torch.autograd import Function

from . import native

ACT_NONE, ACT_LRELU, ACT_RELU, ACT_TANH = 0, 1, 2, 3
CONV, CONVT = 0, 1
CONV_FLAT = CONV | 0x100
BN_MOMENTUM, BN_EPS = 0.1, 1e-5


@dataclass(frozen=True)
class ConvSpec:
    kind: int
    ci: int
    co: int
    k: int
    stride: int = 1
    pad: int = 0
    out_pad: int = 0
    act: int = ACT_NONE
# ... 249 lines not shown
    if len(_lazy_grads) >= 16:
        raise RuntimeError("offer_lazy_grad: 16 gradient placeholders are on offer unclaimed (backward passes outside kernels.backward?)")
    _lazy_grads[g.data_ptr()] = (slices, n, g._version, g.numel(), g)


def claim_lazy_grad(g):
    e = _lazy_grads.pop(g.data_ptr(), None)
    if e is not None and (e[2] != g._version or e[3] != g.numel() or not g.is_contiguous()):
        raise RuntimeError("claim_lazy_grad: a gradient left as split-K slices arrived as something else than its untouched placeholder")
    return e and (e[0], e[1])


class _Tag:
    __slots__ = ("bn_link", "lazy_bn", "fwd_slices", "grad_slices_ok")

    def __init__(self):
        self.bn_link = None
        self.lazy_bn = None
        self.fwd_slices = None
        self.grad_slices_ok = False


_NO_TAG = _Tag()


def tag(t):
    if not hasattr(t, "_ctvae_tag"):
        t._ctvae_tag = _Tag()
    return t._ctvae_tag


def tag_of(t):
    return getattr(t, "_ctvae_tag", _NO_TAG)


def carry_tag(src, view):
    tg = tag_of(src)
    if view is not src and (tg.fwd_slices is not None or tg.grad_slices_ok):
        tag(view).grad_slices_ok = tg.grad_slices_ok
        tag(view).fwd_slices = tg.fwd_slices and tg.fwd_slices[:3] + (_stamp(view),)
    return view


def _handovers_in(x):
    tg, c = tag_of(x), x.is_contiguous()
    return tg.bn_link if c else None, tg.lazy_bn if c else None, tg.grad_slices_ok


def check_fwd_slices(t, fs):
    if fs is not None and not (t.is_contiguous() and _same(t, fs[3])):
        raise RuntimeError("forward split-K slices came with a tensor that is not the untouched placeholder they were made for")
    return fs


def grad_slices_ok(t):
    tag(t).grad_slices_ok = True
    return t


def bn_apply_is_separate(spec, B, H, W) -> bool:
    ws = native.workspace(torch.device("cuda", torch.cuda.current_device()))
    return bool(_geom_query("ctvae_conv_bn_act_apply_is_separate", spec.geom(B, H, W), ws.numel() * 4))


def lazy_bn_input_supported(spec, B, H, W) -> bool:
    return input_transform_supported(spec, B, H, W)


def mark_sole_consumer(x):
    link = tag_of(x).bn_link
    if link is not None:
        link.sole = True
    return x


def _dy_bn_args(dy_bn):
    return (dy_bn[0].data_ptr(), dy_bn[1].data_ptr(), dy_bn[2], native.ptr(dy_bn[3])) if dy_bn is not None else (None, None, 0, None)


def _bn_commit_args(bn_commit):
    return (bn_commit[0].data_ptr(), bn_commit[1].data_ptr(), bn_commit[2]) if bn_commit is not None else (None, None, 0)


def conv_wgrad_raw(x, dy, w_param, b_param, spec: ConvSpec, in_coef=None, in_act=ACT_NONE, dy_bn=None, bn_commit=None):
    B, H, W, _ = x.shape
    ws = native.workspace(x.device)
    gw, gb, acc = _grad_targets(w_param, b_param)
    g = spec.geom(B, H, W)
    native.call("ctvae_conv_wgrad", g[0], x.data_ptr(), dy.data_ptr(), gw.data_ptr(), native.ptr(gb), *g[1:], acc,
                *_coef_ptrs(in_coef, spec.ci), in_act, *_dy_bn_args(dy_bn), *_bn_commit_args(bn_commit),
                ws.data_ptr(), ws.numel() * 4)


_PAIR = True


def _conv_backward_lazy(x, dy, w_param, gw, gb, acc, spec, in_coef, in_act, pixel_major):
    B, H, W, _ = x.shape
    ws = native.workspace(x.device)
    g = spec.geom(B, H, W)
    n = _geom_query("ctvae_conv_backward_lazy_slices", g, 0 if pixel_major else 1, ws.numel() * 4)
    if n <= 1:
        return None
    slices = torch.empty(n * B * H * W * spec.ci, dtype=torch.float32, device=dy.device)
    native.call("ctvae_conv_backward_lazy", g[0], x.data_ptr(), dy.data_ptr(), w_param.data_ptr(), gw.data_ptr(), native.ptr(gb),
                slices.data_ptr(), *g[1:], acc, *_coef_ptrs(in_coef, spec.ci), in_act, pixel_major, ws.data_ptr(), ws.numel() * 4)
    return slices, n


def conv_backward_raw(x, dy, w_param, b_param, spec: ConvSpec, link=None, mask=None, mask_act=ACT_NONE, wino_filters=None,
                      in_coef=None, in_act=ACT_NONE, dy_bn=None, bn_commit=None, grad_slices=False):
    B, H, W, _ = x.shape
    ws = native.workspace(x.device)
    g = spec.geom(B, H, W)
    if wino_filters is not None and wino_filter_floats(spec, B, H, W, ws.numel() // 2) != wino_filters.numel():
        wino_filters = None
    gw, gb, acc = _grad_targets(w_param, b_param)
    dx = torch.empty((B, H, W, spec.ci), dtype=torch.float32, device=dy.device)
    if (link is not None and link.sole and tuple(link.y.shape) == (B, H, W, spec.ci) and mask is None and wino_filters is None
            and dy_bn is None and bn_commit is None):
        lazy = _conv_backward_lazy(x, dy, w_param, gw, gb, acc, spec, in_coef, in_act, 0)
        if lazy is not None:
            link.publish_lazy(dx, *lazy, g)
            return dx
    if grad_slices and link is None and mask is None and wino_filters is None and dy_bn is None and bn_commit is None:
        lazy = _conv_backward_lazy(x, dy, w_param, gw, gb, acc, spec, in_coef, in_act, 1)
        if lazy is not None:
            offer_lazy_grad(dx, *lazy)
            return dx
    part, rows = None, 0
    if link is not None and tuple(link.y.shape) == (B, H, W, spec.ci):
        rows = max(_geom_query("ctvae_conv_backward_bn_rows", g, ws.numel() * 4), 0)
        if rows > 0:
            part = torch.empty(rows * spec.ci * 2, dtype=torch.float32, device=dy.device)
    bn = link if part is not None else None
    coef = torch.empty(7 * spec.ci, dtype=torch.float32, device=dy.device) if bn is not None else None
    cg, cb, cacc = _bn_commit_args(bn_commit)
    if coef is None:
        cg = cb = None
    native.call("ctvae_conv_backward", g[0], x.data_ptr(), dy.data_ptr(), w_param.data_ptr(), gw.data_ptr(), native.ptr(gb),
                dx.data_ptr(), *g[1:], acc, native.ptr(mask), mask_act, native.ptr(wino_filters),
                native.ptr(bn.y if bn else None), native.ptr(bn.mean if bn else None), native.ptr(bn.invstd if bn else None),
                native.ptr(bn.gamma if bn else None), native.ptr(bn.beta if bn else None), bn.act if bn else 0,
                native.ptr(part), rows, native.ptr(coef), cg, cb, cacc,
                *_coef_ptrs(in_coef, spec.ci), in_act, *_dy_bn_args(dy_bn), ws.data_ptr(), ws.numel() * 4)
    if bn is not None:
        bn.publish(dx, part, rows, coef)
    return dx


def wgrad_then_dgrad(x, g, w_param, b_param, spec, need_dgrad, link=None, wino_filters=None, in_coef=None, in_act=ACT_NONE,
                     grad_slices=False):
    if need_dgrad:
        return conv_backward_raw(x, g, w_param, b_param, spec, link=link, wino_filters=wino_filters, in_coef=in_coef, in_act=in_act,
                                 grad_slices=grad_slices)
    conv_wgrad_raw(x, g, w_param, b_param, spec, in_coef=in_coef, in_act=in_act)
    return None


def act_backward_raw(g_out, out, act):
    if act == ACT_NONE:
        return g_out
    g_in = torch.empty_like(out)
    native.call("ctvae_act_backward", g_out.data_ptr(), out.data_ptr(), g_in.data_ptr(), out.numel(), act)
    return g_in


def permute_raw(x, B, C, P, to_nhwc):
    out = torch.empty(x.numel(), dtype=torch.float32, device=x.device)
    native.call("ctvae_permute", x.data_ptr(), out.data_ptr(), B, C, P, 1 if to_nhwc else 0)
    return out


class _ToNHWC(Function):

    @staticmethod
    def forward(ctx, x):
        B, C, H, W = x.shape
        ctx.dims = (B, C, H, W)
        return permute_raw(_c(x), B, C, H * W, True).view(B, H, W, C)

    @staticmethod
    def backward(ctx, g):
        B, C, H, W = ctx.dims
        lazy = claim_lazy_grad(g)
        if lazy is not None:
            out = torch.empty((B, C, H, W), dtype=torch.float32, device=g.device)
            native.call("ctvae_splitk_permute", lazy[0].data_ptr(), lazy[1], out.data_ptr(), B, C, H * W)
            return out
        return permute_raw(_c(g), B, C, H * W, False).view(B, C, H, W)


class LinearToNHWC(Function):

    @staticmethod
    def supported(B, ci, C, P, device):
        return bool(_geom_query("ctvae_linear_pixmajor_supported", (B, ci, C, P), native.workspace(device).numel() * 4))

    @staticmethod
    def forward(ctx, x, w, b, spec, C, h, wd):
        _req_cuda(x, w)
        x = _c(x)
        B = x.shape[0]
        ctx.link_in, _, ctx.x_slices_ok = _handovers_in(x)
        ctx.spec, ctx.w, ctx.b, ctx.dims = spec, w, b, (B, C, h, wd)
        ws = native.workspace(x.device)
        y = torch.empty((B, h, wd, C), dtype=torch.float32, device=x.device)
        native.call("ctvae_linear_pixmajor_forward", x.data_ptr(), w.data_ptr(), native.ptr(b), y.data_ptr(), B, spec.ci, C, h * wd,
                    spec.act, ws.data_ptr(), ws.numel() * 4)
        ctx.save_for_backward(x)
        return y

    @staticmethod
    def backward(ctx, g):
        if g is None:
            return (None,) * 7
        (x,) = ctx.saved_tensors
        B, C, h, wd = ctx.dims
        spec = ctx.spec
        if spec.act != ACT_NONE:
            raise RuntimeError("LinearToNHWC: a fused activation is not differentiated here (decoder_input has none)")
        lazy = claim_lazy_grad(g)
        if lazy is not None:
            g_flat = torch.empty((B, 1, 1, C * h * wd), dtype=torch.float32, device=g.device)
            native.call("ctvae_splitk_permute", lazy[0].data_ptr(), lazy[1], g_flat.data_ptr(), B, C, h * wd)
        else:
            g_flat = permute_raw(_c(g), B, C, h * wd, False).view(B, 1, 1, C * h * wd)
        g_x = wgrad_then_dgrad(x, g_flat, ctx.w, ctx.b, spec, ctx.needs_input_grad[0], ctx.link_in, None, grad_slices=ctx.x_slices_ok)
        return g_x, None, None, None, None, None, None


# ... 254 lines not shown
        ctx.save_for_backward(x, y, save_mean, save_invstd)
        out = y if lazy_out else a
        ctx.link_out = tag(out).bn_link = BNLink(y, save_mean, save_invstd, gamma, beta, bn_act) if training else None
        tag(out).lazy_bn = (coef, bn_act) if lazy_out else None
        return out

    @staticmethod
    def backward(ctx, g_a):
        if not ctx.training:
            raise RuntimeError("backward through eval-mode BatchNorm is not supported on the HIP path")
        spec = ctx.spec
        w, b, gamma, beta = ctx.params
        x, y, save_mean, save_invstd = ctx.saved_tensors
        g_a = _c(g_a)
        in_coef, in_act = ctx.lazy_in if ctx.lazy_in is not None else (None, ACT_NONE)
        gg, gbt, accg = _grad_targets(gamma, beta)
        lazy = ctx.link_out.take_lazy(g_a) if ctx.link_out is not None else None
        if lazy is not None:
            g_y = torch.empty_like(y)
            native.call("ctvae_bn_backward_fused", lazy[0].data_ptr(), lazy[1], *lazy[2], y.data_ptr(), gamma.data_ptr(),
                        beta.data_ptr(), save_mean.data_ptr(), save_invstd.data_ptr(), ctx.bn_act, g_y.data_ptr(), gg.data_ptr(),
                        gbt.data_ptr(), accg)
        else:
            part, rows, coef = ctx.link_out.take(g_a) if ctx.link_out is not None else (None, 0, None)
            if coef is not None:
                part, rows = None, 0
                if not ctx.needs_input_grad[0] and wgrad_bn_apply_mode(spec, x.shape[0], x.shape[1], x.shape[2]) == 2:
                    conv_wgrad_raw(x, g_a, w, b, spec, dy_bn=(y, coef, ctx.bn_act, None), bn_commit=(gg, gbt, accg))
                    return (None,) * 12
            g_y = torch.empty_like(y)
            _bn_backward(g_a, y, (gamma, beta, save_mean, save_invstd), ctx.bn_act, g_y, (gg, gbt, accg), part, rows, coef_in=coef)
        g_x = wgrad_then_dgrad(x, g_y, w, b, spec, ctx.needs_input_grad[0], ctx.link_in, in_coef=in_coef, in_act=in_act,
                               grad_slices=ctx.x_slices_ok)
        return (g_x,) + (None,) * 11


def input_transform_supported(spec: ConvSpec, B, H, W) -> bool:
    return bool(_geom_query("ctvae_conv_input_transform_supported", spec.geom(B, H, W)))


def wgrad_bn_apply_mode(spec: ConvSpec, B, H, W) -> int:
    return int(_geom_query("ctvae_conv_wgrad_bn_apply_supported", spec.geom(B, H, W)))


def wgrad_bn_apply_supported(spec: ConvSpec, B, H, W) -> bool:
    return wgrad_bn_apply_mode(spec, B, H, W) == 1


class ConvBNActConvAct(Function):

    @staticmethod
    def forward(ctx, x, w1, b1, gamma, beta, running_mean, running_var, num_batches_tracked, w2, b2, training, spec1, spec2, bn_act):
        _req_cuda(x, w1, w2, gamma)
        ctx.link_in, ctx.lazy_in, _ = _handovers_in(x)
        x = _c(x)
        y1, _, coef, save_mean, save_invstd = _conv_bn_act_forward(
            x, (w1, b1, gamma, beta), (running_mean, running_var, num_batches_tracked), training, spec1, bn_act, ctx.lazy_in,
            want_a=False, want_coef=True)
        r = conv_forward_raw(y1, w2, b2, spec2, in_coef=coef, in_act=bn_act)
        ctx.act_out = offer_out_act_link(r, spec2.act) if (training and spec2.act != ACT_NONE) else None
        ctx.specs, ctx.bn_act, ctx.training = (spec1, spec2), bn_act, training
        ctx.params = (w1, b1, gamma, beta, w2, b2)
        ctx.save_for_backward(x, y1, r, coef, save_mean, save_invstd)
        return r

    @staticmethod
    def backward(ctx, g_r):
        if not ctx.training:
            raise RuntimeError("backward through eval-mode BatchNorm is not supported on the HIP path")
        spec1, spec2 = ctx.specs
        w1, b1, gamma, beta, w2, b2 = ctx.params
        x, y1, r, coef, save_mean, save_invstd = ctx.saved_tensors
        g_r = _c(g_r)
        if ctx.act_out is not None and ctx.act_out.take(g_r):
            g_pre = g_r
        else:
            g_pre = act_backward_raw(g_r, r, spec2.act) if spec2.act != ACT_NONE else g_r
        C = y1.shape[3]
        bn = (gamma, beta, save_mean, save_invstd)
        link = BNLink(y1, save_mean, save_invstd, gamma, beta, ctx.bn_act)
        grads = _grad_targets(gamma, beta)
        lazy = wgrad_bn_apply_supported(spec1, x.shape[0], x.shape[1], x.shape[2])
        g_y = torch.empty_like(y1)
        g_a = conv_backward_raw(y1, g_pre, w2, b2, spec2, link=link, in_coef=coef, in_act=ctx.bn_act,
                                bn_commit=grads if lazy else None)
        part, rows, c7 = link.take(g_a)
        if c7 is None:
            bcoef = torch.empty(5 * C, dtype=torch.float32, device=x.device) if lazy else None
            _bn_backward(g_a, y1, bn, ctx.bn_act, None if lazy else g_y, grads, part, rows, coef_out=bcoef)
        elif lazy:
            bcoef = c7
        else:
            _bn_backward(g_a, y1, bn, ctx.bn_act, g_y, grads, coef_in=c7)
        in_coef, in_act = ctx.lazy_in if ctx.lazy_in is not None else (None, ACT_NONE)
        if lazy:
            if ctx.needs_input_grad[0]:
                g_x = conv_backward_raw(x, g_a, w1, b1, spec1, link=ctx.link_in, dy_bn=(y1, bcoef, ctx.bn_act, g_y),
                                        in_coef=in_coef, in_act=in_act)
            else:
                conv_wgrad_raw(x, g_a, w1, b1, spec1, dy_bn=(y1, bcoef, ctx.bn_act, g_y), in_coef=in_coef, in_act=in_act)
                g_x = None
        else:
            g_x = wgrad_then_dgrad(x, g_y, w1, b1, spec1, ctx.needs_input_grad[0], ctx.link_in, in_coef=in_coef, in_act=in_act)
        return (g_x,) + (None,) * 13


class ActFn(Function):

    @staticmethod
    def forward(ctx, x, act, aux=None):
        _req_cuda(x)
        x = _c(x)
        ctx.act = act

        def run(t):
            o = torch.empty_like(t)
            native.call("ctvae_act_forward", t.data_ptr(), o.data_ptr(), t.numel(), act)
            return o
        if aux is not None:
            (out,), (out_aux,) = _with_aux(x, _c(aux), run)
            ctx.save_for_backward(out)
            ctx.mark_non_differentiable(out_aux)
            ctx.set_materialize_grads(False)
            return out, out_aux
        out = run(x)
        ctx.save_for_backward(out)
        return out

    @staticmethod
    def backward(ctx, g, *_g_aux):
        if g is None:
            return None, None, None
        (out,) = ctx.saved_tensors
        return act_backward_raw(_c(g), out, ctx.act), None, None


def _rows(t):
    if t.dim() != 2 or t.stride(1) != 1:
        t = t.contiguous()
    return t, t.stride(0)


class SplitHeads(Function):

    @staticmethod
    def forward(ctx, heads, L):
        ctx.L = L
        return heads[:, :L], heads[:, L:]

    @staticmethod
    def backward(ctx, g_mu, g_lv):
        if g_mu is None:
            g_mu = torch.zeros_like(g_lv)
        if g_lv is None:
            g_lv = torch.zeros_like(g_mu)
        return torch.cat([g_mu, g_lv], dim=1), None


class Reparameterize(Function):

    @staticmethod
    def forward(ctx, mu, logvar, eps):
        _req_cuda(mu, logvar, eps)
        mu_, mrs = _rows(mu)
        lv_, lrs = _rows(logvar)
        eps = _c(eps)
        B, L = mu.shape
        z = torch.empty((B, L), dtype=torch.float32, device=mu.device)
        native.call("ctvae_reparam_forward", mu_.data_ptr(), mrs, lv_.data_ptr(), lrs, eps.data_ptr(), z.data_ptr(), B, L)
        ctx.save_for_backward(lv_, eps)
        ctx.lrs = lrs
        return z

    @staticmethod
    def backward(ctx, g_z):
        lv_, eps = ctx.saved_tensors
        g_z = _c(g_z)
# ... 1915 lines not shown
```

ct-vae_amd/native.py:

```python
import ctypes
import os

import torch

_HERE = os.path.dirname(os.path.abspath(__file__))
LIB_PATH = os.environ.get("CTVAE_LIB_OVERRIDE") or os.path.join(_HERE, "lib", "libctvae_hip.so")

_c = ctypes
_fp, _vp, _i, _l, _f, _sz = _c.c_void_p, _c.c_void_p, _c.c_int, _c.c_long, _c.c_float, _c.c_size_t

SIGNATURES = {
    "ctvae_linear_pixmajor_supported": [_i, _i, _i, _i, _sz],
    "ctvae_linear_pixmajor_forward": [_fp, _fp, _fp, _fp, _i, _i, _i, _i, _i, _fp, _sz, _vp],
    "ctvae_conv_forward": [_i, _fp, _fp, _fp, _fp, _fp] + [_i] * 10 + [_fp, _fp, _i, _fp, _fp, _fp, _sz, _vp],
    "ctvae_wino_filters_batch": [_i, _vp, _vp, _vp, _vp, _vp, _vp],
    "ctvae_conv_bn_act_forward": [_i, _fp, _fp, _fp, _fp, _fp, _fp, _fp, _f, _f, _i, _i, _fp, _fp, _fp, _fp, _fp, _fp] + [_i] * 9
                                 + [_fp, _fp, _i, _fp, _sz, _vp],
    "ctvae_conv_dgrad": [_i, _fp, _fp, _fp, _fp, _i, _fp] + [_i] * 9 + [_fp, _fp, _sz, _vp],
    "ctvae_conv_wgrad": [_i, _fp, _fp, _fp, _fp] + [_i] * 10 + [_fp, _fp, _i, _fp, _fp, _i, _fp, _fp, _fp, _i, _fp, _sz, _vp],
    "ctvae_conv_backward": [_i, _fp, _fp, _fp, _fp, _fp, _fp] + [_i] * 10 + [_fp, _i, _fp, _fp, _fp, _fp, _fp, _fp, _i, _fp, _i,
                            _fp, _fp, _fp, _i, _fp, _fp, _i, _fp, _fp, _i, _fp, _fp, _sz, _vp],
    "ctvae_conv_backward_lazy": [_i, _fp, _fp, _fp, _fp, _fp, _fp] + [_i] * 10 + [_fp, _fp, _i, _i, _fp, _sz, _vp],
    "ctvae_bn_backward_fused": [_fp, _i] + [_i] * 10 + [_fp, _fp, _fp, _fp, _fp, _i, _fp, _fp, _fp, _i, _vp],
    "ctvae_bn_forward": [_fp, _i, _i, _fp, _fp, _fp, _fp, _f, _f, _i, _i, _fp, _fp, _fp, _fp, _fp, _sz, _vp],
    "ctvae_bn_backward": [_fp, _fp, _fp, _i, _i, _fp, _fp, _fp, _i, _fp, _fp, _fp, _i, _fp, _i, _fp, _fp, _fp, _sz, _vp],
    "ctvae_permute": [_fp, _fp, _i, _i, _i, _i, _vp],
    "ctvae_crop_resize_u8": [_fp, _fp, _fp, _i, _i, _i, _i, _i, _i, _vp],
    "ctvae_gat_score": [_i, _fp, _fp, _fp, _fp, _fp, _fp, _i, _i, _i, _i, _f, _vp],
    "ctvae_gat_score_backward": [_fp, _fp, _fp, _fp, _fp, _fp, _fp, _fp, _fp, _fp, _i, _i, _i, _i, _f, _vp],
    "ctvae_gat_layer_forward": [_fp, _fp, _i, _fp, _fp, _fp, _fp, _fp, _fp, _i, _fp, _i, _i, _i, _f, _i, _vp],
    "ctvae_gat_layer_backward": [_fp, _fp, _i, _fp, _fp, _fp, _fp, _fp, _fp, _i, _fp, _fp, _fp, _fp, _fp, _fp, _i, _fp, _fp, _fp,
                                 _fp, _i, _i, _i, _i, _f, _i, _vp],
    "ctvae_ct_reg_forward": [_fp, _fp, _fp, _fp, _f, _f, _f, _i, _i, _vp],
    "ctvae_ct_reg_backward": [_fp, _fp, _fp, _fp, _fp, _f, _f, _f, _fp, _fp, _i, _i, _vp],
    "ctvae_ct_blend_softmax_forward": [_fp, _fp, _fp, _l, _i, _i, _vp],
    "ctvae_ct_blend_softmax_backward": [_fp, _fp, _fp, _fp, _fp, _fp, _l, _i, _i, _vp],
    "ctvae_ct_latent_ce_forward": [_fp, _fp, _fp, _l, _i, _vp],
    "ctvae_ct_latent_ce_backward": [_fp, _fp, _fp, _fp, _l, _i, _vp],
    "ctvae_ct_mask_forward": [_fp, _fp, _fp, _fp, _f, _fp, _fp, _fp, _i, _i, _i, _i, _fp, _fp, _fp, _fp, _vp],
    "ctvae_ct_mask_backward": [_fp, _fp, _fp, _fp, _f, _fp, _fp, _fp, _fp, _i, _i, _i, _i, _fp, _fp, _vp],
    "ctvae_ct_blend_forward": [_fp, _fp, _fp, _fp, _l, _vp],
    "ctvae_ct_blend_backward": [_fp, _fp, _fp, _fp, _fp, _fp, _fp, _l, _vp],
    "ctvae_ct_posenc_forward": [_fp, _fp, _fp, _f, _fp, _l, _i, _vp],
    "ctvae_ct_posenc_backward": [_fp, _fp, _f, _fp, _l, _vp],
    "ctvae_one_hot": [_fp, _l, _i, _fp, _vp],
    "ctvae_group_rowsum": [_fp, _l, _i, _i, _i, _i, _fp, _i, _fp, _i, _vp],
    "ctvae_ct_sample_forward": [_fp, _fp, _fp, _fp, _fp, _l, _vp],
    "ctvae_ct_sample_backward": [_fp, _fp, _fp, _fp, _fp, _fp, _l, _vp],
    "ctvae_glinear_forward": [_fp, _i, _i, _i, _i, _vp, _vp, _vp, _vp, _vp, _vp, _fp, _i, _i, _vp],
    "ctvae_glinear_dgrad": [_fp, _i, _i, _i, _vp, _vp, _vp, _vp, _fp, _i, _i, _i, _vp],
    "ctvae_glinear_wgrad": [_fp, _i, _i, _fp, _i, _i, _i, _fp, _i, _i, _fp, _i, _fp, _i, _fp, _sz, _vp],
    "ctvae_pair_mlp_forward": [_fp, _fp, _i, _fp, _fp, _fp, _i, _i, _i, _f, _i, _fp, _vp],
    "ctvae_pair_mlp_backward": [_fp, _fp, _i, _fp, _fp, _fp, _fp, _fp, _i, _fp, _fp, _i, _i, _i, _f, _i, _fp, _vp],
    "ctvae_act_forward": [_fp, _fp, _l, _i, _vp],
    "ctvae_act_backward": [_fp, _fp, _fp, _l, _i, _vp],
    "ctvae_gauss_latent_forward": [_fp, _fp, _fp, _fp, _fp, _i, _i, _fp, _i, _fp, _vp],
    "ctvae_gauss_latent_backward": [_fp, _fp, _fp, _fp, _fp, _fp, _fp, _i, _i, _i, _vp],
    "ctvae_conv_forward_lazy": [_i, _fp, _fp, _fp] + [_i] * 9 + [_fp, _sz, _vp],
    "ctvae_splitk_permute": [_fp, _i, _fp, _i, _i, _i, _vp],
    "ctvae_reparam_forward": [_fp, _l, _fp, _l, _fp, _fp, _i, _i, _vp],
    "ctvae_reparam_backward": [_fp, _fp, _l, _fp, _fp, _fp, _i, _i, _vp],
    "ctvae_loss_forward": [_fp, _fp, _l, _fp, _l, _fp, _l, _i, _i, _f, _fp, _fp, _fp, _sz, _vp],
    "ctvae_loss_forward_grad": [_fp, _fp, _l, _fp, _l, _fp, _l, _i, _i, _f, _fp, _fp, _fp, _fp, _fp, _i, _fp, _sz, _vp],
    "ctvae_mse_backward": [_fp, _fp, _fp, _fp, _l, _i, _vp],
    "ctvae_logcosh_loss_forward": [_fp, _fp, _l, _f, _fp, _l, _fp, _l, _i, _i, _f, _fp, _fp, _sz, _vp],
    "ctvae_logcosh_backward": [_fp, _fp, _fp, _fp, _l, _f, _i, _vp],
    "ctvae_loss_backward": [_fp, _fp, _fp, _fp, _l, _f, _fp, _l, _fp, _l, _fp, _fp, _i, _i, _f, _i, _vp],
    "ctvae_kl_backward": [_fp, _l, _fp, _l, _fp, _fp, _fp, _i, _i, _f, _vp],
    "ctvae_vq_inds": [_fp, _fp, _fp, _i, _i, _i, _i, _i, _vp],
    "ctvae_vq_lookup": [_fp, _fp, _fp, _fp, _fp, _f, _i, _i, _i, _i, _i, _fp, _sz, _vp],
    "ctvae_vq_backward": [_fp, _fp, _fp, _fp, _fp, _fp, _fp, _i, _f, _i, _i, _i, _i, _i, _fp, _sz, _vp],
    "ctvae_gumbel_st_forward": [_fp, _fp, _fp, _fp, _l, _vp],
    "ctvae_gumbel_st_backward": [_fp, _fp, _fp, _fp, _l, _vp],
    "ctvae_gumbel_softmax_forward": [_fp, _fp, _fp, _l, _i, _f, _f, _vp],
    "ctvae_gumbel_softmax_backward": [_fp, _fp, _fp, _l, _i, _f, _vp],
    "ctvae_cat_kl_forward": [_fp, _l, _i, _i, _f, _f, _fp, _fp, _sz, _vp],
    "ctvae_cat_kl_backward": [_fp, _fp, _fp, _l, _i, _i, _f, _f, _vp],
    "ctvae_iw_loss_forward": [_fp, _fp, _l, _i, _i, _fp, _fp, _i, _i, _f, _fp, _fp, _fp, _fp, _vp],
    "ctvae_iw_loss_backward": [_fp, _fp, _l, _i, _i, _fp, _fp, _i, _f, _fp, _fp, _fp, _fp, _fp, _vp],
    "ctvae_l2l1_loss_forward": [_fp, _fp, _l, _fp, _fp, _fp, _sz, _vp],
    "ctvae_l2l1_backward": [_fp, _fp, _fp, _fp, _l, _i, _vp],
    "ctvae_ladder_merge_forward": [_fp, _fp, _fp, _fp, _fp, _i, _i, _fp, _fp, _vp],
    "ctvae_ladder_merge_backward": [_fp, _fp, _fp, _fp, _fp, _fp, _fp, _i, _i, _fp, _fp, _fp, _fp, _vp],
    "ctvae_gamma_reparam_forward": [_fp, _fp, _fp, _f, _fp, _l, _vp],
    "ctvae_gamma_reparam_backward": [_fp, _fp, _fp, _fp, _f, _fp, _fp, _l, _vp],
    "ctvae_gamma_kl_forward": [_fp, _fp, _i, _i, _f, _f, _fp, _fp, _sz, _vp],
    "ctvae_gamma_kl_backward": [_fp, _fp, _fp, _i, _i, _f, _f, _fp, _fp, _vp],
    "ctvae_sigmoid_forward": [_fp, _fp, _l, _vp],
    "ctvae_sigmoid_backward": [_fp, _fp, _fp, _l, _vp],
    "ctvae_tc_forward": [_fp, _fp, _fp, _fp, _i, _i, _fp, _fp, _fp, _fp, _sz, _vp],
    "ctvae_tc_backward": [_fp, _fp, _fp, _fp, _fp, _fp, _fp, _i, _i, _fp, _fp, _fp, _vp],
    "ctvae_vamp_kl_forward": [_fp, _fp, _fp, _fp, _fp, _i, _i, _i, _fp, _fp, _fp, _sz, _vp],
    "ctvae_vamp_kl_backward": [_fp, _fp, _fp, _fp, _fp, _fp, _fp, _i, _i, _i, _fp, _fp, _fp, _fp, _fp, _vp],
    "ctvae_swd_forward": [_fp, _fp, _fp, _i, _i, _i, _f, _f, _fp, _fp, _fp, _sz, _vp],
    "ctvae_mmd_forward": [_fp, _fp, _i, _i, _i, _f, _f, _f, _f, _f, _fp, _fp, _fp, _sz, _vp],
    "ctvae_dip_forward": [_fp, _l, _fp, _l, _i, _i, _f, _f, _fp, _vp],
    "ctvae_dip_backward": [_fp, _fp, _fp, _fp, _i, _i, _vp],
    "ctvae_column_moments": [_fp, _i, _i, _fp, _fp, _fp, _fp, _vp],
    "ctvae_mi_matrix": [_fp, _fp, _fp, _fp, _fp, _i, _i, _i, _fp, _fp, _vp],
    "ctvae_group_var_argmin": [_fp, _fp, _fp, _i, _i, _i, _fp, _fp, _vp],
    "ctvae_image_grid_u8": [_fp, _l, _l, _l, _l, _i, _i, _i, _i, _i, _i, _i, _i, _f, _f, _f, _i, _fp, _sz, _fp, _sz, _vp],
    "ctvae_image_grid_each_u8": [_fp, _l, _l, _l, _l, _i, _i, _i, _i, _i, _i, _i, _i, _f, _f, _f, _i, _fp, _sz, _fp, _sz, _vp],
    "ctvae_action_hits": [_fp, _fp, _i, _i, _fp, _vp],
    "ctvae_graph_accumulate": [_fp, _fp, _fp, _f, _i, _i, _i, _fp, _fp, _fp, _fp, _fp, _fp, _vp],
    "ctvae_heatmap_u8": [_fp, _i, _i, _i, _f, _f, _i, _i, _i, _i, _i, _i, _fp, _i, _fp, _sz, _vp],
    "ctvae_latent_accumulate": [_fp, _l, _fp, _l, _i, _i, _fp, _fp, _fp, _fp, _fp, _fp, _vp],
    "ctvae_gmm_estep": [_fp, _i, _i, _i, _i, _fp, _fp, _fp, _fp, _fp, _fp, _fp, _vp],
    "ctvae_gmm_mstep": [_fp, _fp, _fp, _i, _i, _i, _i, _fp, _fp, _fp, _fp, _fp, _sz, _vp],
    "ctvae_gmm_sample": [_fp, _fp, _i, _i, _i, _i, _fp, _fp, _fp, _fp, _fp, _vp],
    "ctvae_recon_record": [_fp, _fp, _i, _i, _i, _fp, _fp, _fp, _i, _i, _vp],
    "ctvae_recon_worst": [_fp] * 6 + [_i] * 3 + [_fp] * 2 + [_i] * 3 + [_fp] * 5 + [_vp],
    "ctvae_freebits_kl_forward_grad": [_fp, _l, _fp, _l, _i, _i, _fp, _f, _f, _fp, _fp, _fp, _fp, _sz, _vp],
    "ctvae_adam_step": [_fp, _fp, _fp, _fp, _fp, _l, _f, _vp],
    "ctvae_adam_step_clipped": [_fp, _fp, _fp, _fp, _fp, _l, _f, _i, _f, _fp, _fp, _vp],
    "ctvae_adam_mark_members": [_fp, _i, _fp, _i, _vp],
    "ctvae_adam_block_flags": [_fp, _fp, _fp, _i, _fp, _fp, _i, _i, _vp],
    "ctvae_adam_block_flags_local": [_fp, _fp, _fp, _i, _fp, _i, _vp],
    "ctvae_adam_block_flags_finish": [_fp, _fp, _i, _i, _vp],
    "ctvae_adam_step_blocks": [_fp, _fp, _fp, _fp, _fp, _l, _f, _i, _f, _fp, _fp, _fp, _fp, _fp, _fp, _i, _vp],
    "ctvae_grad_accumulate": [_fp, _fp, _l, _i, _vp],
    "ctvae_adam_flags_window": [_fp, _fp, _i, _i, _vp],
    "ctvae_ema_update": [_fp, _fp, _l, _f, _vp],
    "ctvae_buffer_swap": [_fp, _fp, _l, _vp],
    "ctvae_vq_usage": [_fp, _fp, _fp, _i, _i, _i, _i, _vp],
    "ctvae_vq_pool_fill": [_fp, _fp, _l, _i, _l, _vp],
    "ctvae_vq_usage_pool_fill": [_fp, _fp, _fp, _i, _i, _i, _i, _fp, _fp, _l, _i, _l, _vp],
    "ctvae_vq_restart": [_fp, _i, _fp, _i, _i, _fp, _fp, _fp, _fp, _i, _i, _i, _vp],
    "ctvae_vq_restart_gather": [_fp, _i, _fp, _i, _i, _i, _i, _fp, _vp],
    "ctvae_vq_ema_stats": [_fp, _fp, _fp, _fp, _fp, _i, _i, _i, _i, _i, _fp, _sz, _vp],
    "ctvae_vq_ema_update": [_fp, _fp, _fp, _fp, _fp, _i, _i, _i, _f, _f, _vp],
    "ctvae_vq_lookup_commit": [_fp, _fp, _fp, _fp, _fp, _f, _i, _i, _i, _i, _i, _fp, _sz, _vp],
    "ctvae_grad_segment_stats": [_fp, _l, _f, _f, _fp, _i, _fp, _fp, _fp, _i, _fp, _fp, _fp, _fp, _fp, _fp, _fp, _fp, _fp, _i, _vp],
    "ctvae_grad_segment_hist": [_fp, _l, _f, _fp, _i, _fp, _fp, _i, _fp, _fp, _vp],
    "ctvae_mssim_forward": [_fp, _fp, _fp, _fp, _fp, _fp, _fp, _i, _i, _i, _i, _vp],
    "ctvae_mssim_backward": [_fp, _fp, _fp, _fp, _fp, _fp, _i, _i, _i, _i, _vp],
    "ctvae_defer_begin": [_fp, _sz],
    "ctvae_defer_flush": [_vp],
}
_RESTYPES = {
    "ctvae_version": _c.c_char_p,
    "ctvae_arch": _c.c_char_p,
    "ctvae_error_string": _c.c_char_p,
    "ctvae_workspace_bytes": _c.c_size_t,
    "ctvae_prof_enable": None,
    "ctvae_prof_calibrate": None,
    "ctvae_prof_report": _c.c_size_t,
    "ctvae_conv_backward_bn_rows": _c.c_int,
    "ctvae_conv_backward_lazy_slices": _c.c_int,
    "ctvae_conv_forward_lazy_slices": _c.c_int,
    "ctvae_conv_bn_act_apply_is_separate": _c.c_int,
    "ctvae_winograd_enable": _c.c_int,
    "ctvae_conv_wino_filter_floats": _c.c_size_t,
    "ctvae_dip_state_floats": _c.c_size_t,
    "ctvae_adam_state_floats": _c.c_size_t,
    "ctvae_grad_clip_workspace_floats": _c.c_size_t,
    "ctvae_grad_accumulate_pass_floats": _c.c_size_t,
    "ctvae_vq_usage_pass_indices": _c.c_size_t,
    "ctvae_vq_ema_supported": _c.c_int,
    "ctvae_grad_segment_chunk_floats": _c.c_size_t,
    "ctvae_mssim_part_floats": _c.c_size_t,
    "ctvae_freebits_workspace_bytes": _c.c_size_t,
    "ctvae_gmm_mstep_slabs": _c.c_int,
    "ctvae_gmm_mstep_workspace_bytes": _c.c_size_t,
    "ctvae_glinear_wgrad_ws_bytes": _c.c_size_t,
    "ctvae_conv_input_transform_supported": _c.c_int,
    "ctvae_conv_wgrad_bn_apply_supported": _c.c_int,
}
EXPORTS = sorted(list(SIGNATURES) + list(_RESTYPES))

_lib = None


def load():
    global _lib
    if _lib is not None:
        return _lib
    if not os.path.exists(LIB_PATH):
        raise RuntimeError(
            f"{LIB_PATH} is missing: build it with `python -m ctvae_amd.build` (hipcc, gfx950). "
            "There is no CPU/PyTorch fallback for the ctvae hot path.")
    try:
        lib = ctypes.CDLL(LIB_PATH)
    except OSError as e:
        raise RuntimeError(f"cannot load {LIB_PATH}: {e}") from e
    for name, argtypes in SIGNATURES.items():
        fn = getattr(lib, name, None)
        if fn is None:
            raise RuntimeError(f"{LIB_PATH} does not export {name} (stale build?)")
        fn.argtypes = argtypes
        fn.restype = _c.c_int
    for name, res in _RESTYPES.items():
        fn = getattr(lib, name, None)
        if fn is None:
            raise RuntimeError(f"{LIB_PATH} does not export {name} (stale build?)")
        fn.restype = res
        fn.argtypes = {"ctvae_error_string": [_c.c_int], "ctvae_prof_enable": [_c.c_int],
                       "ctvae_prof_calibrate": [_c.c_void_p, _c.c_int],
                       "ctvae_prof_report": [_c.c_char_p, _c.c_size_t],
                       "ctvae_conv_backward_bn_rows": [_c.c_int] * 10 + [_c.c_size_t],
                       "ctvae_conv_backward_lazy_slices": [_c.c_int] * 11 + [_c.c_size_t],
                       "ctvae_conv_forward_lazy_slices": [_c.c_int] * 10 + [_c.c_size_t],
                       "ctvae_conv_bn_act_apply_is_separate": [_c.c_int] * 10 + [_c.c_size_t],
                       "ctvae_winograd_enable": [_c.c_int],
                       "ctvae_dip_state_floats": [_c.c_int, _c.c_int],
                       "ctvae_vq_ema_supported": [_c.c_int] * 3,
                       "ctvae_freebits_workspace_bytes": [_c.c_int],
                       "ctvae_gmm_mstep_slabs": [_c.c_int] * 4,
                       "ctvae_gmm_mstep_workspace_bytes": [_c.c_int] * 4,
                       "ctvae_glinear_wgrad_ws_bytes": [_c.c_int] * 5,
                       "ctvae_conv_wino_filter_floats": [_c.c_int] * 10 + [_c.c_size_t],
                       "ctvae_conv_input_transform_supported": [_c.c_int] * 10,
                       "ctvae_conv_wgrad_bn_apply_supported": [_c.c_int] * 10}.get(name, [])
    if lib.ctvae_arch() != b"gfx950":
        raise RuntimeError("libctvae_hip.so was not built for gfx950")
    _lib = lib
    return lib


def check(code: int, what: str):
    if code != 0:
        msg = load().ctvae_error_string(int(code)).decode()
        raise RuntimeError(f"{what} failed: {msg} (code {code})")


def stream_ptr() -> int:
    return torch.cuda.current_stream().cuda_stream


def ptr(t):
    return None if t is None else t.data_ptr()


_workspaces = {}


def workspace(device) -> torch.Tensor:
    key = (device.index if device.index is not None else torch.cuda.current_device(), torch.cuda.current_stream().cuda_stream)
    ws = _workspaces.get(key)
    if ws is None:
        n = load().ctvae_workspace_bytes()
        ws = torch.empty(n // 4, dtype=torch.float32, device=device)
        _workspaces[key] = ws
    return ws


def call(name: str, *args):
    lib = load()
    check(getattr(lib, name)(*args, stream_ptr()), name)


_wino_on = None


def winograd_enable(on: bool) -> bool:
    global _wino_on
    prev = bool(load().ctvae_winograd_enable(1 if on else 0))
    _wino_on = bool(on)
    return prev


def winograd_enabled() -> bool:
    global _wino_on
    if _wino_on is None:
        lib = load()
        _wino_on = bool(lib.ctvae_winograd_enable(1))
        lib.ctvae_winograd_enable(1 if _wino_on else 0)
    return _wino_on


def prof_enable(on, detailed: bool = False):
    load().ctvae_prof_enable((2 if detailed else 1) if on else 0)


def prof_calibrate(n: int = 64):
    load().ctvae_prof_calibrate(stream_ptr(), n)


def prof_report() -> dict:
    lib = load()
    buf = ctypes.create_string_buffer(1 << 16)
    lib.ctvae_prof_report(buf, len(buf))
    out = {}
    for line in buf.value.decode().splitlines():
        name, cnt, ms, fl, by = line.split("\t")
        out[name] = dict(count=int(cnt), ms=float(ms), flops=float(fl), bytes=float(by))
    return out
```

include/ctvae_hip.h:

```cpp
#ifndef CTVAE_HIP_H
#define CTVAE_HIP_H
#include <stddef.h>
#include <stdint.h>

#ifdef __cplusplus
extern "C" {
#endif

#define CTVAE_ACT_NONE 0
#define CTVAE_ACT_LRELU 1
#define CTVAE_ACT_RELU 2
#define CTVAE_ACT_TANH 3

#define CTVAE_CONV 0
#define CTVAE_CONVT 1
#define CTVAE_W_CI_TAP 0x100

const char* ctvae_version(void);
const char* ctvae_arch(void);
const char* ctvae_error_string(int code);
size_t ctvae_workspace_bytes(void);

int ctvae_conv_forward(int kind, const float* x, const float* w, const float* bias, const float* add, float* y, int B,
                       int H, int W, int Ci, int Co, int k, int stride, int pad, int out_pad, int act, const float* in_scale,
                       const float* in_shift, int in_act, float* wino_dgrad_filters_out, const float* wino_fwd_filters, float* ws,
                       size_t ws_bytes, void* stream);
int ctvae_linear_pixmajor_supported(int B, int Ci, int C, int P, size_t ws_bytes);
int ctvae_linear_pixmajor_forward(const float* x, const float* w, const float* bias, float* y, int B, int Ci, int C, int P, int act,
                                  float* ws, size_t ws_bytes, void* stream);
int ctvae_wino_filters_batch(int n, const float* const* w, float* const* fwd_filters, float* const* dgrad_filters, const int* Ci,
                             const int* Co, void* stream);
size_t ctvae_conv_wino_filter_floats(int kind, int B, int H, int W, int Ci, int Co, int k, int stride, int pad, int out_pad,
                                     size_t ws_bytes);
int ctvae_conv_input_transform_supported(int kind, int B, int H, int W, int Ci, int Co, int k, int stride, int pad,
                                         int out_pad);

int ctvae_conv_bn_act_apply_is_separate(int kind, int B, int H, int W, int Ci, int Co, int k, int stride, int pad, int out_pad,
                                        size_t ws_bytes);
int ctvae_conv_bn_act_forward(int kind, const float* x, const float* w, const float* bias, const float* gamma,
                              const float* beta, float* running_mean, float* running_var, float momentum, float eps,
                              int training, int act, float* y, float* a_out, float* save_mean, float* save_invstd,
                              float* scale_shift_out, int64_t* num_batches_tracked, int B, int H, int W, int Ci, int Co, int k,
                              int stride, int pad, int out_pad, const float* in_scale, const float* in_shift, int in_act,
                              float* ws, size_t ws_bytes, void* stream);

int ctvae_conv_dgrad(int kind, const float* dy, const float* w, const float* add, const float* mask, int mask_act,
                     float* dx, int B, int H, int W, int Ci, int Co, int k, int stride, int pad, int out_pad,
                     const float* wino_filters, float* ws, size_t ws_bytes, void* stream);

int ctvae_conv_wgrad(int kind, const float* x, const float* dy, float* dw, float* dbias, int B, int H, int W, int Ci,
                     int Co, int k, int stride, int pad, int out_pad, int accumulate, const float* in_scale,
                     const float* in_shift, int in_act, const float* dy_bn_y, const float* dy_bn_coef, int dy_bn_act,
                     float* gy_out, float* bn_dgamma, float* bn_dbeta, int bn_accumulate, float* ws, size_t ws_bytes,
                     void* stream);
int ctvae_conv_backward_bn_rows(int kind, int B, int H, int W, int Ci, int Co, int k, int stride, int pad, int out_pad,
                                size_t ws_bytes);
int ctvae_conv_backward(int kind, const float* x, const float* dy, const float* w, float* dw, float* dbias, float* dx, int B,
                        int H, int W, int Ci, int Co, int k, int stride, int pad, int out_pad, int accumulate, const float* mask,
                        int mask_act, const float* wino_filters, const float* bn_y, const float* bn_mean,
                        const float* bn_invstd, const float* bn_gamma, const float* bn_beta, int bn_act, float* bn_part,
                        int bn_part_rows, float* bn_coef_out, float* bn_dgamma, float* bn_dbeta, int bn_accumulate,
                        const float* in_scale, const float* in_shift, int in_act,
                        const float* dy_bn_y, const float* dy_bn_coef, int dy_bn_act, float* gy_out, float* ws, size_t ws_bytes,
                        void* stream);

int ctvae_conv_backward_lazy_slices(int kind, int B, int H, int W, int Ci, int Co, int k, int stride, int pad, int out_pad,
                                    int for_bn, size_t ws_bytes);
int ctvae_conv_backward_lazy(int kind, const float* x, const float* dy, const float* w, float* dw, float* dbias, float* dx_slices,
                             int B, int H, int W, int Ci, int Co, int k, int stride, int pad, int out_pad, int accumulate,
                             const float* in_scale, const float* in_shift, int in_act, int pixel_major, float* ws, size_t ws_bytes,
                             void* stream);
int ctvae_bn_backward_fused(const float* g_a_slices, int slices, int kind, int B, int H, int W, int Ci, int Co, int k, int stride,
                            int pad, int out_pad, const float* y, const float* gamma, const float* beta, const float* save_mean,
                            const float* save_invstd, int act, float* g_y, float* dgamma, float* dbeta, int accumulate, void* stream);

int ctvae_conv_wgrad_bn_apply_supported(int kind, int B, int H, int W, int Ci, int Co, int k, int stride, int pad,
                                        int out_pad);

int ctvae_bn_forward(const float* y, int R, int C, const float* gamma, const float* beta, float* running_mean,
                     float* running_var, float momentum, float eps, int training, int act, float* out,
                     float* save_mean, float* save_invstd, int64_t* num_batches_tracked, float* ws, size_t ws_bytes,
                     void* stream);
int ctvae_bn_backward(const float* g_a, const float* beta, const float* y, int R, int C, const float* gamma,
                      const float* save_mean, const float* save_invstd, int act, float* g_y, float* dgamma,
                      float* dbeta, int accumulate, const float* part_in, int part_rows, float* coef_out,
                      const float* coef_in, float* ws, size_t ws_bytes, void* stream);

int ctvae_pair_mlp_forward(const float* u, const float* v, int ld, const float* w2, const float* b2, float* out, int B, int N,
                           int H, float slope, int per_sample, const int32_t* row_of, void* stream);
int ctvae_pair_mlp_backward(const float* u, const float* v, int ld, const float* w2, const float* out, const float* g_out,
                            float* d_u, float* d_v, int ldd, float* d_w2_part, float* d_b2_part, int B, int N, int H, float slope,
                            int per_sample, const int32_t* row_of, void* stream);

int ctvae_gat_score(int mode, const float* xl, const float* xr, const float* attr, const float* we, const float* att, float* out,
                    int B, int N, int H, int C, float slope, void* stream);
int ctvae_gat_score_backward(const float* xl, const float* xr, const float* attr, const float* we, const float* att,
                             const float* g, float* d_xl, float* d_xr, float* d_att_part, float* d_we_part, int B, int N, int H,
                             int C, float slope, void* stream);

int ctvae_gat_layer_forward(const float* xl, const float* xr, int ld, const float* adj, const float* we, const float* att,
                            const float* bias, const int32_t* head_map, float* out, int ldo, float* alpha, int B, int Hs, int C,
                            float slope, int act, void* stream);
int ctvae_gat_layer_backward(const float* xl, const float* xr, int ld, const float* adj, const float* we, const float* att,
                             const float* bias, const int32_t* head_map, const float* out, int ldo, const float* alpha,
                             const float* g_out, float* dS, float* dattr, float* d_xl, float* d_xr, int ldd, float* d_bias_part,
                             float* d_att_part, float* d_we_part, float* d_adj, int accumulate_dadj, int B, int Hs, int C,
                             float slope, int act, void* stream);

int ctvae_glinear_forward(const float* x, int ldx, int K, int nseg, int N, const float* const* W, const int* ldw,
                          const int64_t* w_gstride, const float* const* bias, const int* b_gstride,
                          const int32_t* const* group, float* y, int ldy, int B, void* stream);
int ctvae_glinear_dgrad(const float* dy, int ldy, int nseg, int N, const float* const* W, const int* ldw,
                        const int64_t* w_gstride, const int32_t* const* group, float* dx, int ldx, int K, int B, void* stream);
size_t ctvae_glinear_wgrad_ws_bytes(int G, int N, int K, int B, int grouped);
int ctvae_glinear_wgrad(const float* x, int ldx, int K, const float* dy, int ldy, int col0, int N, const int32_t* group, int G,
                        int B, float* dW, int ldo, float* dbias, int accumulate, float* ws, size_t ws_bytes, void* stream);

int ctvae_ct_blend_forward(const float* s0, const float* s1, const float* mask, float* out, long rows, void* stream);
int ctvae_ct_blend_backward(const float* g, const float* s0, const float* s1, const float* mask, float* g0, float* g1, float* g_mask,
                            long rows, void* stream);
int ctvae_ct_posenc_forward(const float* x, const float* pe, const float* keep, float scale, float* out, long n, int sd,
                            void* stream);
int ctvae_ct_posenc_backward(const float* g, const float* keep, float scale, float* g_x, long n, void* stream);
int ctvae_one_hot(const int64_t* inds, long n, int N, float* out, void* stream);
int ctvae_group_rowsum(const float* parts, long mat_stride, int nmat, int rows, int C, int ld, const int32_t* group, int G, float* out,
                       int accumulate, void* stream);

int ctvae_ct_reg_forward(const float* adj, const float* graph, const float* uniform, float* part4, float ckl, float cgs, float cpt,
                         int B, int N, void* stream);
int ctvae_ct_reg_backward(const float* adj, const float* graph, const float* uniform, const float* part4, const float* g_loss,
                          float ckl, float cgs, float cpt, float* d_adj, float* d_graph, int B, int N, void* stream);
int ctvae_ct_blend_softmax_forward(const float* y, const float* mask, float* probs, long R, int Hs, int D, void* stream);
int ctvae_ct_blend_softmax_backward(const float* g, const float* probs, const float* y, const float* mask, float* dy, float* dmask,
                                    long R, int Hs, int D, void* stream);
int ctvae_ct_latent_ce_forward(const float* probs, const int64_t* target, float* row_loss, long R, int D, void* stream);
int ctvae_ct_latent_ce_backward(const float* probs, const int64_t* target, const float* g_loss, float* d_probs, long R, int D,
                                void* stream);

int ctvae_ct_mask_forward(const float* x, const float* action, const float* pe, const float* keep, float scale, const float* W,
                          const float* bias, const float* expo, int B, int S, int D, int A, float* inter, float* p, float* sample,
                          float* soft, void* stream);
int ctvae_ct_mask_backward(const float* x, const float* action, const float* pe, const float* keep, float scale, const float* inter,
                           const float* p, const float* soft, const float* g, int B, int S, int D, int A, float* dWp, float* dbp,
                           void* stream);
int ctvae_ct_sample_forward(const float* p, const float* expo, float* sample, float* soft, float* weighted, long n, void* stream);
int ctvae_ct_sample_backward(const float* g_sample, const float* g_weighted, const float* p, const float* soft, const float* sample,
                             float* g_p, long n, void* stream);

int ctvae_permute(const float* in, float* out, int B, int C, int P, int to_nhwc, void* stream);
int ctvae_act_forward(const float* in, float* out, long n, int act, void* stream);
int ctvae_act_backward(const float* g_out, const float* out, float* g_in, long n, int act, void* stream);

int ctvae_gauss_latent_forward(float* heads, const float* eps_in, const uint64_t* rng, float* eps_out, float* z, int B, int L,
                               const float* head_slices, int slices, const float* head_bias, void* stream);
int ctvae_gauss_latent_backward(const float* g_mu, const float* g_logvar, const float* g_z, const float* heads, const float* eps,
                                float* g_heads, uint64_t* rng_bump, int B, int L, int g_z_slices, void* stream);
int ctvae_conv_forward_lazy_slices(int kind, int B, int H, int W, int Ci, int Co, int k, int stride, int pad, int out_pad,
                                   size_t ws_bytes);
int ctvae_conv_forward_lazy(int kind, const float* x, const float* w, float* y_slices, int B, int H, int W, int Ci, int Co, int k,
                            int stride, int pad, int out_pad, float* ws, size_t ws_bytes, void* stream);
// ... 218 lines not shown
```

Before: 89090 images/s.

## Recompute final-layer dgrad inside upconv wgrad instead of materializing it

For the last upconv followed by the 3-channel output conv, the output conv's backward now runs without writing dX (a no-store variant of the fused image kernel). The upconv's wgrad/dgrad kernel instead recomputes that gradient on the fly from the small 3-channel gradient and the output-conv weights using MFMA in shared memory. This is meant to remove a full 32-channel activation-gradient write and re-read at the highest resolution. The cost is extra MFMA work and larger shared-memory use in the upconv kernel, plus extra code paths that must match the geometry checks.

```diff
diff --git a/ct-vae_amd/csrc/api.hip b/ct-vae_amd/csrc/api.hip
--- a/ct-vae_amd/csrc/api.hip
+++ b/ct-vae_amd/csrc/api.hip
@@ -444,6 +444,18 @@
 }
 
 static thread_local int g_lazy_pixel_major = 0;
+static thread_local int g_no_dx = 0;
+static thread_local const DyRecompute* g_recompute = nullptr;
+
+static bool recompute_geom(const ConvGeom& g1, int kind2, int Co2, int k2, int stride2, int pad2, int out_pad2, DyRecompute* rc) {
+  if (!upconv_wgrad_supported(g1) || !conv_kind_ok(kind2)) return false;
+  ConvGeom g2;
+  if (conv_geom(g2, kind2, 2, g1.B, g1.sH, g1.sW, g1.sC, Co2, k2, stride2, pad2, out_pad2)) return false;
+  if (!img_dgrad_supported(g2) || g2.B != g1.B || g2.sH != g1.sH || g2.sW != g1.sW) return false;
+  if (rc != nullptr)
+    for (int t = 0; t < 9; ++t) { rc->tdy[t] = g2.taps[0][t].dy; rc->tdx[t] = g2.taps[0][t].dx; rc->twt[t] = g2.taps[0][t].wtap; }
+  return true;
+}
 
 static int conv_backward_impl(int kind, const float* x, const float* dy, const float* w, float* dw, float* dbias, float* dx, int B,
                         int H, int W, int Ci, int Co, int k, int stride, int pad, int out_pad, int accumulate, const float* mask,
@@ -453,7 +465,12 @@
                         const float* in_scale, const float* in_shift, int in_act,
                         const float* dy_bn_y, const float* dy_bn_coef, int dy_bn_act, float* gy_out, float* ws, size_t ws_bytes,
                         void* stream, float* dx_slices) {
-  if (!x || !dy || !w || !dw || (!dx && !dx_slices) || !ws || !conv_kind_ok(kind)) return kErrBadArg;
+  const bool no_dx = g_no_dx != 0;
+  const DyRecompute* const recompute = g_recompute;
+  g_no_dx = 0;
+  g_recompute = nullptr;
+  if (!x || (!dy && !recompute) || !w || !dw || (!dx && !dx_slices && !no_dx) || !ws || !conv_kind_ok(kind)) return kErrBadArg;
+  if (recompute != nullptr && (dy_bn_y == nullptr || gy_out == nullptr)) return kErrBadArg;
   const bool bn = bn_part != nullptr;
   if (bn_coef_out != nullptr && !bn) return kErrBadArg;
   if ((bn_dgamma != nullptr) != (bn_dbeta != nullptr) || (bn_dgamma != nullptr && bn_coef_out == nullptr)) return kErrBadArg;
@@ -486,10 +503,17 @@
     ctx.dgrad_chunks = pl.splitk > 1 ? (kmax + pl.splitk - 1) / pl.splitk : kmax;
   }
   const InXform xf{in_scale, in_shift, in_act};
-  const DyXform dyx{dy_bn_y, dy_bn_coef, gy_out, dy_bn_act};
+  DyXform dyx{dy_bn_y, dy_bn_coef, gy_out, dy_bn_act};
+  dyx.rc = recompute;
   int rc;
-  if (bn && bn_act != ACT_TANH && x == bn_y && in_scale != nullptr && in_act == bn_act && mask == nullptr && dy_bn_y == nullptr &&
-      img_conv_supported(gw) && img_dgrad_supported(gd) && img_backward_fused_ws_floats(gd) <= half_floats) {
+  const bool img_fused = bn && bn_act != ACT_TANH && x == bn_y && in_scale != nullptr && in_act == bn_act && mask == nullptr &&
+                         dy_bn_y == nullptr && img_conv_supported(gw) && img_dgrad_supported(gd) &&
+                         img_backward_fused_ws_floats(gd) <= half_floats;
+  if ((no_dx && !img_fused) || (recompute != nullptr && !upconv_wgrad_supported(gw))) {
+    pair_ctx() = nullptr;
+    return kErrBadArg;
+  }
+  if (img_fused) {
     float *part = nullptr, *pb = nullptr;
     int np = 0;
     const BnBwdFuse f{bn_y, bn_mean, bn_invstd, bn_gamma, bn_beta, bn_act, bn_part};
@@ -533,6 +557,67 @@
                             ws_bytes, stream, nullptr);
 }
 
+int ctvae_conv_backward_nodx(int kind, const float* x, const float* dy, const float* w, float* dw, float* dbias, int B, int H,
+                             int W, int Ci, int Co, int k, int stride, int pad, int out_pad, int accumulate, const float* bn_y,
+                             const float* bn_mean, const float* bn_invstd, const float* bn_gamma, const float* bn_beta, int bn_act,
+                             float* bn_part, int bn_part_rows, float* bn_coef_out, float* bn_dgamma, float* bn_dbeta,
+                             int bn_accumulate, const float* in_scale, const float* in_shift, int in_act, float* ws, size_t ws_bytes,
+                             void* stream) {
+  g_no_dx = 1;
+  return conv_backward_impl(kind, x, dy, w, dw, dbias, nullptr, B, H, W, Ci, Co, k, stride, pad, out_pad, accumulate, nullptr, 0,
+                            nullptr, bn_y, bn_mean, bn_invstd, bn_gamma, bn_beta, bn_act, bn_part, bn_part_rows, bn_coef_out,
+                            bn_dgamma, bn_dbeta, bn_accumulate, in_scale, in_shift, in_act, nullptr, nullptr, 0, nullptr, ws, ws_bytes,
+                            stream, nullptr);
+}
+
+int ctvae_conv_recompute_supported(int kind, int B, int H, int W, int Ci, int Co, int k, int stride, int pad, int out_pad, int kind2,
+                                   int Co2, int k2, int stride2, int pad2, int out_pad2) {
+  if (!conv_kind_ok(kind)) return 0;
+  ConvGeom g;
+  if (conv_geom(g, kind, 0, B, H, W, Ci, Co, k, stride, pad, out_pad)) return 0;
+  return recompute_geom(g, kind2, Co2, k2, stride2, pad2, out_pad2, nullptr) ? 1 : 0;
+}
+
+int ctvae_conv_backward_recompute(int kind, const float* x, const float* g_pre, const float* w2, const float* w, float* dw,
+                                  float* dbias, float* dx, int B, int H, int W, int Ci, int Co, int k, int stride, int pad, int out_pad,
+                                  int accumulate, const float* bn_y, const float* bn_mean, const float* bn_invstd,
+                                  const float* bn_gamma, const float* bn_beta, int bn_act, float* bn_part, int bn_part_rows,
+                                  float* bn_coef_out, float* bn_dgamma, float* bn_dbeta, int bn_accumulate, const float* in_scale,
+                                  const float* in_shift, int in_act, const float* dy_bn_y, const float* dy_bn_coef, int dy_bn_act,
+                                  float* gy_out, int kind2, int Co2, int k2, int stride2, int pad2, int out_pad2, float* ws,
+                                  size_t ws_bytes, void* stream) {
+  if (!g_pre || !w2 || !dx || !dy_bn_y || !dy_bn_coef || !gy_out || !conv_kind_ok(kind)) return kErrBadArg;
+  ConvGeom g;
+  DyRecompute rc{g_pre, w2, {}, {}, {}};
+  if (conv_geom(g, kind, 0, B, H, W, Ci, Co, k, stride, pad, out_pad)) return kErrBadArg;
+  if (!recompute_geom(g, kind2, Co2, k2, stride2, pad2, out_pad2, &rc)) return kErrBadArg;
+  g_recompute = &rc;
+  return conv_backward_impl(kind, x, nullptr, w, dw, dbias, dx, B, H, W, Ci, Co, k, stride, pad, out_pad, accumulate, nullptr, 0,
+                            nullptr, bn_y, bn_mean, bn_invstd, bn_gamma, bn_beta, bn_act, bn_part, bn_part_rows, bn_coef_out,
+                            bn_dgamma, bn_dbeta, bn_accumulate, in_scale, in_shift, in_act, dy_bn_y, dy_bn_coef, dy_bn_act, gy_out, ws,
+                            ws_bytes, stream, nullptr);
+}
+
+int ctvae_conv_wgrad_recompute(int kind, const float* x, const float* g_pre, const float* w2, float* dw, float* dbias, int B, int H,
+                               int W, int Ci, int Co, int k, int stride, int pad, int out_pad, int accumulate, const float* in_scale,
+                               const float* in_shift, int in_act, const float* dy_bn_y, const float* dy_bn_coef, int dy_bn_act,
+                               float* gy_out, int kind2, int Co2, int k2, int stride2, int pad2, int out_pad2, float* ws,
+                               size_t ws_bytes, void* stream) {
+  if (!x || !g_pre || !w2 || !dw || !ws || !dy_bn_y || !dy_bn_coef || !gy_out || !conv_kind_ok(kind)) return kErrBadArg;
+  if ((in_scale != nullptr) != (in_shift != nullptr)) return kErrBadArg;
+  ConvGeom g;
+  DyRecompute rc{g_pre, w2, {}, {}, {}};
+  if (conv_geom(g, kind, 0, B, H, W, Ci, Co, k, stride, pad, out_pad)) return kErrBadArg;
+  if (!recompute_geom(g, kind2, Co2, k2, stride2, pad2, out_pad2, &rc)) return kErrBadArg;
+  const InXform xf{in_scale, in_shift, in_act};
+  DyXform dyx{dy_bn_y, dy_bn_coef, gy_out, dy_bn_act};
+  dyx.rc = &rc;
+  float* wws = defer_wgrad_ws(ws, ws_bytes / sizeof(float));
+  const int rcode = launch_wgrad(g, x, nullptr, dw, dbias, wws, ws_bytes, accumulate, (hipStream_t)stream, &xf, &dyx);
+  defer_wgrad_done();
+  return rcode;
+}
+
 int ctvae_conv_backward_lazy_slices(int kind, int B, int H, int W, int Ci, int Co, int k, int stride, int pad, int out_pad,
                                     int for_bn, size_t ws_bytes) {
   if (!conv_kind_ok(kind)) return 0;
diff --git a/ct-vae_amd/csrc/common.hpp b/ct-vae_amd/csrc/common.hpp
--- a/ct-vae_amd/csrc/common.hpp
+++ b/ct-vae_amd/csrc/common.hpp
@@ -137,6 +137,12 @@
   int act;
 };
 
+struct DyRecompute {
+  const float* g_pre;
+  const float* w2;
+  int tdy[9], tdx[9], twt[9];
+};
+
 struct DyXform {
   const float* y;
   const float* coef;
@@ -145,6 +151,7 @@
   float* dgamma = nullptr;
   float* dbeta = nullptr;
   int bn_accumulate = 0;
+  const DyRecompute* rc = nullptr;
 };
 
 struct WinoFilters {
diff --git a/ct-vae_amd/csrc/image.hip b/ct-vae_amd/csrc/image.hip
--- a/ct-vae_amd/csrc/image.hip
+++ b/ct-vae_amd/csrc/image.hip
@@ -503,6 +503,7 @@
   }
 }
 
+template <bool STORE>
 __global__ __launch_bounds__(256, 4) void img_bwd_fused_kernel(const ImgArgs a, float* __restrict__ wpart, float* __restrict__ wpbias) {
   kernarg_warm<sizeof(ImgArgs) + 16>();
   const float bn_slope = act_slope(a.bn_act);
@@ -513,7 +514,7 @@
   const int tid = threadIdx.x, lane = tid & 63, wave = tid >> 6, li = lane & 31, lh = lane >> 5;
   const __amdgpu_buffer_rsrc_t rG = rsrc(a.dY, (long)a.B * a.H * a.W * NO * 4);
   const long obytes = (long)a.B * a.H * a.W * C * 4;
-  const __amdgpu_buffer_rsrc_t rO = rsrc(a.out, obytes);
+  const __amdgpu_buffer_rsrc_t rO = rsrc(a.out, STORE ? obytes : 0);
   const __amdgpu_buffer_rsrc_t rY = rsrc(a.bn_y, obytes);
 
   int koff[14];
@@ -585,8 +586,10 @@
       const float* gp = &sG[((ly + 1) * PW + li + 1) * 4];
 #pragma unroll
       for (int s = 0; s < 14; ++s) acc = __builtin_amdgcn_mfma_f32_32x32x2f32(gp[koff[s]], bw[s], acc, 0, 0, 0);
-#pragma unroll
-      for (int r = 0; r < 16; ++r) st1(rO, rowoff + (unsigned)((8 * (r >> 2) + 4 * lh + (r & 3)) * C) * 4u, acc[r]);
+      if constexpr (STORE) {
+#pragma unroll
+        for (int r = 0; r < 16; ++r) st1(rO, rowoff + (unsigned)((8 * (r >> 2) + 4 * lh + (r & 3)) * C) * 4u, acc[r]);
+      }
       const float* gw = &sG[ly * PW * 4 + wlane];
 #pragma unroll
       for (int r = 0; r < 16; ++r) {
@@ -999,8 +1002,10 @@
   const int nwg = img_dgrad_rows(g);
   float* part = ws;
   float* pb = want_bias ? ws + (size_t)nwg * NT * C * NO : nullptr;
-  ProfScope ps("img_bwd_fused_kernel", st, 4.0 * a.ntiles * TH * TW * NT * C * NO, 4.0 * a.ntiles * TH * TW * (C * 2 + NO));
-  hipLaunchKernelGGL(img_bwd_fused_kernel, dim3(nwg), dim3(256), 0, st, a, part, pb);
+  ProfScope ps("img_bwd_fused_kernel", st, 4.0 * a.ntiles * TH * TW * NT * C * NO,
+               4.0 * a.ntiles * TH * TW * (C * (dX != nullptr ? 2 : 1) + NO));
+  if (dX != nullptr) hipLaunchKernelGGL(img_bwd_fused_kernel<true>, dim3(nwg), dim3(256), 0, st, a, part, pb);
+  else hipLaunchKernelGGL(img_bwd_fused_kernel<false>, dim3(nwg), dim3(256), 0, st, a, part, pb);
   CTVAE_LAUNCH_CHECK();
   *part_out = part;
   *pbias_out = pb;
diff --git a/ct-vae_amd/csrc/upconv.hip b/ct-vae_amd/csrc/upconv.hip
--- a/ct-vae_amd/csrc/upconv.hip
+++ b/ct-vae_amd/csrc/upconv.hip
@@ -12,6 +12,7 @@
 constexpr int LDA = 36, C = 32, NT = 9, NCLS = 4, MAXT = 4;
 constexpr int NLD = (NP * 8 + 255) / 256;
 constexpr unsigned kOOBu = 0x80000000u;
+constexpr int GPH = 2 * TH + 2, GPW = 2 * TW + 2, GNP = GPH * GPW , GNLD = (GNP + 255) / 256 , NO = 3, NJ = 27;
 
 struct UpArgs {
   const float* X;
@@ -25,6 +26,9 @@
   const float* dy_coef;
   float* gy_out;
   int dy_act;
+  const float* rc_g;
+  const float* rc_w;
+  int rc_tdy[NT], rc_tdx[NT], rc_twt[NT];
   const float* xf_scale;
   const float* xf_shift;
   int xf_act;
@@ -269,17 +273,19 @@
   static constexpr int first = CLS == 0 ? 0 : (CLS == 1 ? 1 : (CLS == 2 ? 3 : 5));
 };
 
-template <bool FUSED>
-__global__ __launch_bounds__(256, 1) void up_wgrad_kernel(const UpArgs a) {
+template <int MODE>
+__device__ __forceinline__ void up_wgrad_body(const UpArgs& a) {
+  constexpr bool FUSED = MODE >= 1, RECOMP = MODE == 2;
   kernarg_warm<sizeof(UpArgs)>();
   __shared__ __attribute__((aligned(16))) float sA[NP * LDA];
-  __shared__ __attribute__((aligned(16))) float sR[4 * C * C];
+  __shared__ __attribute__((aligned(16))) float sR[RECOMP ? GNP * 4 : 4 * C * C];
+  static_assert(GNP * 4 >= 4 * C * C, "the gradient patch is the larger tenant");
   __shared__ float sB[4 * C];
   const int tid = threadIdx.x, lane = tid & 63, wave = tid >> 6, li = lane & 31, lh = lane >> 5;
   const __amdgpu_buffer_rsrc_t rX = rsrc(a.X, (long)a.B * a.H * a.W * C * 4);
   const int OH = 2 * a.H, OW = 2 * a.W;
   const long obytes = (long)a.B * OH * OW * C * 4;
-  const __amdgpu_buffer_rsrc_t rG = rsrc(a.dY, obytes);
+  const __amdgpu_buffer_rsrc_t rG = RECOMP ? rsrc(a.rc_g, (long)a.B * OH * OW * NO * 4) : rsrc(a.dY, obytes);
   const __amdgpu_buffer_rsrc_t rYb = rsrc(a.dy_y, FUSED ? obytes : 0);
   const __amdgpu_buffer_rsrc_t rGY = rsrc(a.gy_out, FUSED ? obytes : 0);
   const float k1 = FUSED ? a.dy_coef[li] : 0.f, k2 = FUSED ? a.dy_coef[C + li] : 0.f, k3 = FUSED ? a.dy_coef[2 * C + li] : 0.f;
@@ -290,6 +296,22 @@
   const f32x4 xsh = xf ? *reinterpret_cast<const f32x4*>(a.xf_shift + 4 * (tid & 7)) : f32x4{0.f, 0.f, 0.f, 0.f};
   const float xns = a.xf_act == ACT_LRELU ? kLeaky : (a.xf_act == ACT_RELU ? 0.f : 1.f);
 
+  int koff[RECOMP ? 14 : 1];
+  float bw[RECOMP ? 14 : 1];
+  const int qli = (li & ~7) + 2 * (li & 3) + ((li >> 2) & 1);
+  if constexpr (RECOMP) {
+#pragma unroll
+    for (int s = 0; s < 14; ++s) {
+      const int k0 = 2 * s, k1 = 2 * s + 1;
+      const int t0 = k0 / 3, c0 = k0 % 3, t1 = (k1 < NJ ? k1 : 0) / 3, c1 = (k1 < NJ ? k1 : 0) % 3;
+      const int o0 = (a.rc_tdy[t0] * GPW + a.rc_tdx[t0]) * 4 + c0, o1 = (a.rc_tdy[t1] * GPW + a.rc_tdx[t1]) * 4 + c1;
+      const float w0 = a.rc_w[(a.rc_twt[t0] * C + li) * NO + c0];
+      const float w1 = k1 < NJ ? a.rc_w[(a.rc_twt[t1] * C + li) * NO + c1] : 0.f;
+      koff[s] = lh ? (k1 < NJ ? o1 : 0) : o0;
+      bw[s] = lh ? w1 : w0;
+    }
+  }
+
   f32x16 acc[NT];
 #pragma unroll
   for (int t = 0; t < NT; ++t)
@@ -301,12 +323,37 @@
   for (int tile = blockIdx.x; tile < a.ntiles; tile += gridDim.x) {
     const TileXY cur = tile_xy(a, tile);
     CTVAE_PH(up, 1, 1);
-#pragma unroll
-    for (int h = 0; h < 2; ++h) {
-      f32x4 v[NLD / 2];
-#pragma unroll
-      for (int j = 0; j < NLD / 2; ++j) {
-        const int e = tid + 256 * (j + h * (NLD / 2));
+    constexpr int YS = 2;
+    float yv[RECOMP ? YS : 1][16];
+    unsigned boff[YS];
+    auto y_issue = [&](auto n_c) {
+      constexpr int N = decltype(n_c)::value;
+      const int ly = wave + 4 * (N / 4);
+      boff[N % YS] = (unsigned)((((cur.b * OH + 2 * (cur.y0 + ly) + a.cpy[N % 4]) * OW + 2 * cur.x0 + a.cpx[N % 4] + 2 * lh) * C + li)) * 4u;
+#pragma unroll
+      for (int r = 0; r < 16; ++r) yv[N % YS][r] = ld1(rYb, boff[N % YS] + (unsigned)(4 * r * C) * 4u);
+    };
+    float gq[RECOMP ? GNLD : 1][NO];
+    if constexpr (RECOMP) {
+      y_issue(std::integral_constant<int, 0>{});
+#pragma unroll
+      for (int j = 0; j < GNLD; ++j) {
+        const int pp = tid + 256 * j;
+        const int py = pp / GPW, px = pp - py * GPW;
+        const int iy = 2 * cur.y0 - 1 + py, ix = 2 * cur.x0 - 1 + px;
+        const bool ok = pp < GNP && (unsigned)iy < (unsigned)OH && (unsigned)ix < (unsigned)OW;
+        const unsigned off = (unsigned)(((cur.b * OH + iy) * OW + ix) * NO) * 4u;
+#pragma unroll
+        for (int n = 0; n < NO; ++n) gq[j][n] = ld1(rG, ok ? off + 4u * n : kOOBu);
+      }
+    }
+    constexpr int NR = RECOMP ? 1 : 2, NPR = NLD / NR;
+#pragma unroll
+    for (int h = 0; h < NR; ++h) {
+      f32x4 v[NPR];
+#pragma unroll
+      for (int j = 0; j < NPR; ++j) {
+        const int e = tid + 256 * (j + h * (NPR));
         const int pp = e >> 3, c4 = e & 7;
         const int py = (pp * 1986) >> 16, px = pp - py * PW;
         const int iy = cur.y0 + py, ix = cur.x0 + px;
@@ -315,8 +362,8 @@
       }
       if (xf) {
 #pragma unroll
-        for (int j = 0; j < NLD / 2; ++j) {
-          const int e = tid + 256 * (j + h * (NLD / 2));
+        for (int j = 0; j < NPR; ++j) {
+          const int e = tid + 256 * (j + h * (NPR));
           const int pp = e >> 3;
           const int py = (pp * 1986) >> 16, px = pp - py * PW;
           const float inside = (cur.y0 + py < a.H && cur.x0 + px < a.W) ? 1.f : 0.f;
@@ -328,14 +375,90 @@
         }
       }
 #pragma unroll
-      for (int j = 0; j < NLD / 2; ++j) {
-        const int e = tid + 256 * (j + h * (NLD / 2));
+      for (int j = 0; j < NPR; ++j) {
+        const int e = tid + 256 * (j + h * (NPR));
         if (e < NP * 8) *reinterpret_cast<f32x4*>(&sA[(e >> 3) * LDA + 4 * (e & 7)]) = v[j];
       }
     }
+    if constexpr (RECOMP) {
+#pragma unroll
+      for (int j = 0; j < GNLD; ++j) {
+        const int pp = tid + 256 * j;
+        if (pp < GNP)
+#pragma unroll
+          for (int n = 0; n < NO; ++n) sR[pp * 4 + n] = gq[j][n];
+      }
+    }
     __syncthreads();
 
     CTVAE_PH(up, 1, 2);
+    if constexpr (RECOMP) {
+      f32x16 ga[2];
+      auto gp_of = [&](int n) {
+        const int ly = wave + 4 * (n / 4), c = n % 4;
+        return &sR[((2 * ly + a.cpy[c] + 1) * GPW + 2 * qli + a.cpx[c] + 1) * 4];
+      };
+      auto run_blk = [&](auto n_c) {
+        constexpr int N = decltype(n_c)::value;
+        constexpr int CLS = N % 4, slot = N % YS, gs = N % 2, gn = (N + 1) % 2;
+        constexpr bool more = N + 1 < 8;
+        using CI = ClsInfo<CLS>;
+        const int ly = wave + 4 * (N / 4);
+        if constexpr (N + YS - 1 < 8) y_issue(std::integral_constant<int, N + YS - 1>{});
+        const float* gpn = gp_of(more ? N + 1 : N);
+        int xo[CI::ntaps];
+#pragma unroll
+        for (int t = 0; t < CI::ntaps; ++t) xo[t] = ((ly + a.tdy[CLS][t]) * PW + lh + a.tdx[CLS][t]) * LDA + li;
+        float xa[CI::ntaps], xb[CI::ntaps];
+#pragma unroll
+        for (int t = 0; t < CI::ntaps; ++t) xa[t] = sA[xo[t]];
+        float gcur = 0.f, gnxt = 0.f;
+        if constexpr (more) {
+          gcur = gpn[koff[0]];
+#pragma unroll
+          for (int r = 0; r < 16; ++r) ga[gn][r] = 0.f;
+        }
+#pragma unroll
+        for (int r = 0; r < 16; ++r) {
+          if (r + 1 < 16) {
+#pragma unroll
+            for (int t = 0; t < CI::ntaps; ++t) xb[t] = sA[xo[t] + 2 * (r + 1) * LDA];
+          }
+          if constexpr (more) {
+            if (r + 1 < 14) gnxt = gpn[koff[r + 1]];
+          }
+          const float yy = yv[slot][r];
+          float d = ga[gs][r];
+          const float g1 = (yy * ksc + ksh) > 0.f ? d : d * nslope;
+          d = k1 * g1 + k2 * yy + k3;
+          st1(rGY, boff[slot] + (unsigned)(4 * r * C) * 4u, d);
+          bsum += d;
+#pragma unroll
+          for (int t = 0; t < CI::ntaps; ++t)
+            acc[CI::first + t] = __builtin_amdgcn_mfma_f32_32x32x2f32(xa[t], d, acc[CI::first + t], 0, 0, 0);
+          if constexpr (more) {
+            if (r < 14) ga[gn] = __builtin_amdgcn_mfma_f32_32x32x2f32(gcur, bw[r], ga[gn], 0, 0, 0);
+          }
+#pragma unroll
+          for (int t = 0; t < CI::ntaps; ++t) xa[t] = xb[t];
+          gcur = gnxt;
+          __builtin_amdgcn_sched_barrier(0);
+        }
+      };
+      if constexpr (YS > 2) y_issue(std::integral_constant<int, 1>{});
+      {
+        const float* gp0 = gp_of(0);
+#pragma unroll
+        for (int r = 0; r < 16; ++r) ga[0][r] = 0.f;
+#pragma unroll
+        for (int s = 0; s < 14; ++s) ga[0] = __builtin_amdgcn_mfma_f32_32x32x2f32(gp0[koff[s]], bw[s], ga[0], 0, 0, 0);
+      }
+#define UPW_BLK(N_) run_blk(std::integral_constant<int, N_>{});
+      UPW_BLK(0) UPW_BLK(1) UPW_BLK(2) UPW_BLK(3)
+      CTVAE_PH(up, 1, 3);
+      UPW_BLK(4) UPW_BLK(5) UPW_BLK(6) UPW_BLK(7)
+#undef UPW_BLK
+    } else {
     float dv[3][8], yv[FUSED ? 3 : 1][FUSED ? 8 : 1];
     auto step_off = [&](int ly, int c, int h) {
       return (unsigned)((((cur.b * OH + 2 * (cur.y0 + ly) + a.cpy[c]) * OW + 2 * cur.x0 + a.cpx[c] + 2 * (16 * h + lh)) * C + li)) * 4u;
@@ -399,6 +522,7 @@
     CTVAE_PH(up, 1, 3);
     UPW_STEP(8) UPW_STEP(9) UPW_STEP(10) UPW_STEP(11) UPW_STEP(12) UPW_STEP(13) UPW_STEP(14) UPW_STEP(15)
 #undef UPW_STEP
+    }
     CTVAE_PH(up, 1, 4);
     __syncthreads();
   }
@@ -427,6 +551,17 @@
   CTVAE_PH(up, 1, 5);
 }
 
+template <bool FUSED>
+__global__ __launch_bounds__(256, 1) void up_wgrad_kernel(const UpArgs a) {
+  up_wgrad_body<FUSED ? 1 : 0>(a);
+}
+struct Recompute {};
+template <typename Mode>
+__global__ __launch_bounds__(256, 1) void up_wgrad_kernel(const UpArgs a) {
+  static_assert(std::is_same<Mode, Recompute>::value, "modes 0 / 1 are up_wgrad_kernel<false> / <true>");
+  up_wgrad_body<2>(a);
+}
+
 void fill(UpArgs& a, const ConvGeom& g) {
   a.B = g.B; a.H = g.gH; a.W = g.gW;
   a.tiles_y = g.gH / TH; a.tiles_x = g.gW / TW;
@@ -501,11 +636,27 @@
   }
   if (dyx != nullptr && dyx->y != nullptr && dyx->act != ACT_NONE && dyx->act != ACT_RELU && dyx->act != ACT_LRELU) return kErrBadArg;
   if (dyx != nullptr && dyx->y != nullptr) { a.dy_y = dyx->y; a.dy_coef = dyx->coef; a.gy_out = dyx->gy_out; a.dy_act = dyx->act; }
+  const DyRecompute* rc = dyx != nullptr ? dyx->rc : nullptr;
+  if (rc != nullptr) {
+    if (a.dy_y == nullptr || a.dy_coef == nullptr || a.gy_out == nullptr || rc->g_pre == nullptr || rc->w2 == nullptr) return kErrBadArg;
+    for (int c = 0; c < NCLS; ++c)
+      if (a.cpy[c] < 0 || a.cpy[c] > 1 || a.cpx[c] < 0 || a.cpx[c] > 1) return kErrBadArg;
+    for (int t = 0; t < NT; ++t) {
+      if (rc->tdy[t] < -1 || rc->tdy[t] > 1 || rc->tdx[t] < -1 || rc->tdx[t] > 1 || rc->twt[t] < 0 || rc->twt[t] >= NT) return kErrBadArg;
+      a.rc_tdy[t] = rc->tdy[t]; a.rc_tdx[t] = rc->tdx[t]; a.rc_twt[t] = rc->twt[t];
+    }
+    a.rc_g = rc->g_pre; a.rc_w = rc->w2;
+  } else if (dY == nullptr) {
+    return kErrBadArg;
+  }
   const int nwg = upconv_rows(g);
   a.out = ws;
   a.pbias = want_bias ? ws + (size_t)nwg * NT * C * C : nullptr;
-  ProfScope ps("up_wgrad_kernel", st, 2.0 * a.ntiles * TH * TW * NT * C * C, 4.0 * a.ntiles * TH * TW * C * 5.0);
-  if (a.dy_y != nullptr) hipLaunchKernelGGL(up_wgrad_kernel<true>, dim3(nwg), dim3(256), 0, st, a);
+  const double px_bytes = rc != nullptr ? 4.0 * (C * 9.0 + 4.0 * NO) : 4.0 * C * 5.0;
+  const double px_flops = 2.0 * NT * C * C + (rc != nullptr ? 2.0 * 4 * NJ * C : 0.0);
+  ProfScope ps("up_wgrad_kernel", st, a.ntiles * TH * TW * px_flops, a.ntiles * TH * TW * px_bytes);
+  if (rc != nullptr) hipLaunchKernelGGL(up_wgrad_kernel<Recompute>, dim3(nwg), dim3(256), 0, st, a);
+  else if (a.dy_y != nullptr) hipLaunchKernelGGL(up_wgrad_kernel<true>, dim3(nwg), dim3(256), 0, st, a);
   else hipLaunchKernelGGL(up_wgrad_kernel<false>, dim3(nwg), dim3(256), 0, st, a);
   CTVAE_LAUNCH_CHECK();
   *part_out = a.out;
diff --git a/ct-vae_amd/csrc/wgrad.hip b/ct-vae_amd/csrc/wgrad.hip
--- a/ct-vae_amd/csrc/wgrad.hip
+++ b/ct-vae_amd/csrc/wgrad.hip
@@ -349,6 +349,7 @@
                    ws_bytes / sizeof(float) >= (size_t)512 * (27 * 32 + 32);
   if (dyx != nullptr && dyx->y != nullptr && !up && !(enc && dyx->gy_out == nullptr)) return kErrBadArg;
   if (dyx != nullptr && dyx->y != nullptr && up && dyx->gy_out == nullptr) return kErrBadArg;
+  if (dyx != nullptr && dyx->rc != nullptr && (!up || dyx->y == nullptr)) return kErrBadArg;
   if (up) {
     float *part = nullptr, *pb = nullptr;
     int np = 0;
diff --git a/ct-vae_amd/kernels.py b/ct-vae_amd/kernels.py
--- a/ct-vae_amd/kernels.py
+++ b/ct-vae_amd/kernels.py
@@ -355,11 +355,17 @@
     return (bn_commit[0].data_ptr(), bn_commit[1].data_ptr(), bn_commit[2]) if bn_commit is not None else (None, None, 0)
 
 
-def conv_wgrad_raw(x, dy, w_param, b_param, spec: ConvSpec, in_coef=None, in_act=ACT_NONE, dy_bn=None, bn_commit=None):
+def conv_wgrad_raw(x, dy, w_param, b_param, spec: ConvSpec, in_coef=None, in_act=ACT_NONE, dy_bn=None, bn_commit=None,
+                   recompute=None):
     B, H, W, _ = x.shape
     ws = native.workspace(x.device)
     gw, gb, acc = _grad_targets(w_param, b_param)
     g = spec.geom(B, H, W)
+    if recompute is not None:
+        native.call("ctvae_conv_wgrad_recompute", g[0], x.data_ptr(), dy.data_ptr(), recompute[0].data_ptr(), gw.data_ptr(),
+                    native.ptr(gb), *g[1:], acc, *_coef_ptrs(in_coef, spec.ci), in_act, *_dy_bn_args(dy_bn),
+                    *_conv2_args(recompute[1]), ws.data_ptr(), ws.numel() * 4)
+        return
     native.call("ctvae_conv_wgrad", g[0], x.data_ptr(), dy.data_ptr(), gw.data_ptr(), native.ptr(gb), *g[1:], acc,
                 *_coef_ptrs(in_coef, spec.ci), in_act, *_dy_bn_args(dy_bn), *_bn_commit_args(bn_commit),
                 ws.data_ptr(), ws.numel() * 4)
@@ -382,7 +388,7 @@
 
 
 def conv_backward_raw(x, dy, w_param, b_param, spec: ConvSpec, link=None, mask=None, mask_act=ACT_NONE, wino_filters=None,
-                      in_coef=None, in_act=ACT_NONE, dy_bn=None, bn_commit=None, grad_slices=False):
+                      in_coef=None, in_act=ACT_NONE, dy_bn=None, bn_commit=None, grad_slices=False, recompute=None):
     B, H, W, _ = x.shape
     ws = native.workspace(x.device)
     g = spec.geom(B, H, W)
@@ -411,6 +417,17 @@
     cg, cb, cacc = _bn_commit_args(bn_commit)
     if coef is None:
         cg = cb = None
+    if recompute is not None:
+        native.call("ctvae_conv_backward_recompute", g[0], x.data_ptr(), dy.data_ptr(), recompute[0].data_ptr(), w_param.data_ptr(),
+                    gw.data_ptr(), native.ptr(gb), dx.data_ptr(), *g[1:], acc,
+                    native.ptr(bn.y if bn else None), native.ptr(bn.mean if bn else None), native.ptr(bn.invstd if bn else None),
+                    native.ptr(bn.gamma if bn else None), native.ptr(bn.beta if bn else None), bn.act if bn else 0,
+                    native.ptr(part), rows, native.ptr(coef), cg, cb, cacc,
+                    *_coef_ptrs(in_coef, spec.ci), in_act, *_dy_bn_args(dy_bn), *_conv2_args(recompute[1]),
+                    ws.data_ptr(), ws.numel() * 4)
+        if bn is not None:
+            bn.publish(dx, part, rows, coef)
+        return dx
     native.call("ctvae_conv_backward", g[0], x.data_ptr(), dy.data_ptr(), w_param.data_ptr(), gw.data_ptr(), native.ptr(gb),
                 dx.data_ptr(), *g[1:], acc, native.ptr(mask), mask_act, native.ptr(wino_filters),
                 native.ptr(bn.y if bn else None), native.ptr(bn.mean if bn else None), native.ptr(bn.invstd if bn else None),
@@ -420,6 +437,31 @@
     if bn is not None:
         bn.publish(dx, part, rows, coef)
     return dx
+
+
+def _conv2_args(spec2: ConvSpec):
+    return (spec2.kind, spec2.co, spec2.k, spec2.stride, spec2.pad, spec2.out_pad)
+
+
+def conv_recompute_supported(spec: ConvSpec, spec2: ConvSpec, B, H, W) -> bool:
+    return spec2.ci == spec.co and bool(_geom_query("ctvae_conv_recompute_supported", spec.geom(B, H, W), *_conv2_args(spec2)))
+
+
+def conv_backward_nodx_raw(x, dy, w_param, b_param, spec: ConvSpec, link, in_coef, in_act, bn_commit):
+    B, H, W, _ = x.shape
+    ws = native.workspace(x.device)
+    g = spec.geom(B, H, W)
+    rows = max(_geom_query("ctvae_conv_backward_bn_rows", g, ws.numel() * 4), 0)
+    if rows <= 0 or tuple(link.y.shape) != (B, H, W, spec.ci) or in_coef is None:
+        return None
+    gw, gb, acc = _grad_targets(w_param, b_param)
+    part = torch.empty(rows * spec.ci * 2, dtype=torch.float32, device=dy.device)
+    coef = torch.empty(7 * spec.ci, dtype=torch.float32, device=dy.device)
+    native.call("ctvae_conv_backward_nodx", g[0], x.data_ptr(), dy.data_ptr(), w_param.data_ptr(), gw.data_ptr(), native.ptr(gb),
+                *g[1:], acc, link.y.data_ptr(), link.mean.data_ptr(), link.invstd.data_ptr(), link.gamma.data_ptr(),
+                link.beta.data_ptr(), link.act, part.data_ptr(), rows, coef.data_ptr(), *_bn_commit_args(bn_commit),
+                *_coef_ptrs(in_coef, spec.ci), in_act, ws.data_ptr(), ws.numel() * 4)
+    return coef
 
 
 def wgrad_then_dgrad(x, g, w_param, b_param, spec, need_dgrad, link=None, wino_filters=None, in_coef=None, in_act=ACT_NONE,
@@ -840,6 +882,18 @@
         grads = _grad_targets(gamma, beta)
         lazy = wgrad_bn_apply_supported(spec1, x.shape[0], x.shape[1], x.shape[2])
         g_y = torch.empty_like(y1)
+        in_coef, in_act = ctx.lazy_in if ctx.lazy_in is not None else (None, ACT_NONE)
+        if lazy and conv_recompute_supported(spec1, spec2, x.shape[0], x.shape[1], x.shape[2]):
+            c7 = conv_backward_nodx_raw(y1, g_pre, w2, b2, spec2, link, coef, ctx.bn_act, grads)
+            if c7 is not None:
+                dy_bn, rc = (y1, c7, ctx.bn_act, g_y), (w2, spec2)
+                if ctx.needs_input_grad[0]:
+                    g_x = conv_backward_raw(x, g_pre, w1, b1, spec1, link=ctx.link_in, dy_bn=dy_bn, in_coef=in_coef, in_act=in_act,
+                                            recompute=rc)
+                else:
+                    conv_wgrad_raw(x, g_pre, w1, b1, spec1, dy_bn=dy_bn, in_coef=in_coef, in_act=in_act, recompute=rc)
+                    g_x = None
+                return (g_x,) + (None,) * 13
         g_a = conv_backward_raw(y1, g_pre, w2, b2, spec2, link=link, in_coef=coef, in_act=ctx.bn_act,
                                 bn_commit=grads if lazy else None)
         part, rows, c7 = link.take(g_a)
@@ -850,7 +904,6 @@
             bcoef = c7
         else:
             _bn_backward(g_a, y1, bn, ctx.bn_act, g_y, grads, coef_in=c7)
-        in_coef, in_act = ctx.lazy_in if ctx.lazy_in is not None else (None, ACT_NONE)
         if lazy:
             if ctx.needs_input_grad[0]:
                 g_x = conv_backward_raw(x, g_a, w1, b1, spec1, link=ctx.link_in, dy_bn=(y1, bcoef, ctx.bn_act, g_y),
diff --git a/ct-vae_amd/native.py b/ct-vae_amd/native.py
--- a/ct-vae_amd/native.py
+++ b/ct-vae_amd/native.py
@@ -20,6 +20,12 @@
     "ctvae_conv_wgrad": [_i, _fp, _fp, _fp, _fp] + [_i] * 10 + [_fp, _fp, _i, _fp, _fp, _i, _fp, _fp, _fp, _i, _fp, _sz, _vp],
     "ctvae_conv_backward": [_i, _fp, _fp, _fp, _fp, _fp, _fp] + [_i] * 10 + [_fp, _i, _fp, _fp, _fp, _fp, _fp, _fp, _i, _fp, _i,
                             _fp, _fp, _fp, _i, _fp, _fp, _i, _fp, _fp, _i, _fp, _fp, _sz, _vp],
+    "ctvae_conv_backward_nodx": [_i, _fp, _fp, _fp, _fp, _fp] + [_i] * 10 + [_fp, _fp, _fp, _fp, _fp, _i, _fp, _i, _fp, _fp, _fp, _i,
+                                 _fp, _fp, _i, _fp, _sz, _vp],
+    "ctvae_conv_backward_recompute": [_i, _fp, _fp, _fp, _fp, _fp, _fp, _fp] + [_i] * 10 + [_fp, _fp, _fp, _fp, _fp, _i, _fp, _i, _fp,
+                                      _fp, _fp, _i, _fp, _fp, _i, _fp, _fp, _i, _fp] + [_i] * 6 + [_fp, _sz, _vp],
+    "ctvae_conv_wgrad_recompute": [_i, _fp, _fp, _fp, _fp, _fp] + [_i] * 10 + [_fp, _fp, _i, _fp, _fp, _i, _fp] + [_i] * 6
+                                   + [_fp, _sz, _vp],
     "ctvae_conv_backward_lazy": [_i, _fp, _fp, _fp, _fp, _fp, _fp] + [_i] * 10 + [_fp, _fp, _i, _i, _fp, _sz, _vp],
     "ctvae_bn_backward_fused": [_fp, _i] + [_i] * 10 + [_fp, _fp, _fp, _fp, _fp, _i, _fp, _fp, _fp, _i, _vp],
     "ctvae_bn_forward": [_fp, _i, _i, _fp, _fp, _fp, _fp, _f, _f, _i, _i, _fp, _fp, _fp, _fp, _fp, _sz, _vp],
@@ -165,6 +171,7 @@
     "ctvae_glinear_wgrad_ws_bytes": _c.c_size_t,
     "ctvae_conv_input_transform_supported": _c.c_int,
     "ctvae_conv_wgrad_bn_apply_supported": _c.c_int,
+    "ctvae_conv_recompute_supported": _c.c_int,
 }
 EXPORTS = sorted(list(SIGNATURES) + list(_RESTYPES))
 
@@ -210,7 +217,8 @@
                        "ctvae_glinear_wgrad_ws_bytes": [_c.c_int] * 5,
                        "ctvae_conv_wino_filter_floats": [_c.c_int] * 10 + [_c.c_size_t],
                        "ctvae_conv_input_transform_supported": [_c.c_int] * 10,
-                       "ctvae_conv_wgrad_bn_apply_supported": [_c.c_int] * 10}.get(name, [])
+                       "ctvae_conv_wgrad_bn_apply_supported": [_c.c_int] * 10,
+                       "ctvae_conv_recompute_supported": [_c.c_int] * 16}.get(name, [])
     if lib.ctvae_arch() != b"gfx950":
         raise RuntimeError("libctvae_hip.so was not built for gfx950")
     _lib = lib
diff --git a/include/ctvae_hip.h b/include/ctvae_hip.h
--- a/include/ctvae_hip.h
+++ b/include/ctvae_hip.h
@@ -76,6 +76,28 @@
 
 int ctvae_conv_wgrad_bn_apply_supported(int kind, int B, int H, int W, int Ci, int Co, int k, int stride, int pad,
                                         int out_pad);
+
+int ctvae_conv_recompute_supported(int kind, int B, int H, int W, int Ci, int Co, int k, int stride, int pad, int out_pad, int kind2,
+                                   int Co2, int k2, int stride2, int pad2, int out_pad2);
+int ctvae_conv_backward_nodx(int kind, const float* x, const float* dy, const float* w, float* dw, float* dbias, int B, int H,
+                             int W, int Ci, int Co, int k, int stride, int pad, int out_pad, int accumulate, const float* bn_y,
+                             const float* bn_mean, const float* bn_invstd, const float* bn_gamma, const float* bn_beta, int bn_act,
+                             float* bn_part, int bn_part_rows, float* bn_coef_out, float* bn_dgamma, float* bn_dbeta,
+                             int bn_accumulate, const float* in_scale, const float* in_shift, int in_act, float* ws, size_t ws_bytes,
+                             void* stream);
+int ctvae_conv_backward_recompute(int kind, const float* x, const float* g_pre, const float* w2, const float* w, float* dw,
+                                  float* dbias, float* dx, int B, int H, int W, int Ci, int Co, int k, int stride, int pad, int out_pad,
+                                  int accumulate, const float* bn_y, const float* bn_mean, const float* bn_invstd,
+                                  const float* bn_gamma, const float* bn_beta, int bn_act, float* bn_part, int bn_part_rows,
+                                  float* bn_coef_out, float* bn_dgamma, float* bn_dbeta, int bn_accumulate, const float* in_scale,
+                                  const float* in_shift, int in_act, const float* dy_bn_y, const float* dy_bn_coef, int dy_bn_act,
+                                  float* gy_out, int kind2, int Co2, int k2, int stride2, int pad2, int out_pad2, float* ws,
+                                  size_t ws_bytes, void* stream);
+int ctvae_conv_wgrad_recompute(int kind, const float* x, const float* g_pre, const float* w2, float* dw, float* dbias, int B, int H,
+                               int W, int Ci, int Co, int k, int stride, int pad, int out_pad, int accumulate, const float* in_scale,
+                               const float* in_shift, int in_act, const float* dy_bn_y, const float* dy_bn_coef, int dy_bn_act,
+                               float* gy_out, int kind2, int Co2, int k2, int stride2, int pad2, int out_pad2, float* ws,
+                               size_t ws_bytes, void* stream);
 
 int ctvae_bn_forward(const float* y, int R, int C, const float* gamma, const float* beta, float* running_mean,
                      float* running_var, float momentum, float eps, int training, int act, float* out,
```

New measurement: 91190 images/s (median of 6 runs). +2.4%, better.
